# KieDani/UpliftingTableTennis

Hardware: AMD Instinct MI355X
Metric: frames/sec end-to-end (detect+uplift), 1280x720 (higher is better)
Workload: dtype bf16

## Files before the change

### upliftingtabletennis_amd/csrc/conv.h

```cpp
#pragma once
#include "common.h"
#include "wasb_graph.h"

namespace ttup {

struct PackedConv {
    int cout = 0, cin_total = 0, c0 = 0, k = 1, stride = 1, ck = 32;
    void*  w_dev = nullptr;
    void*  w3_dev = nullptr;
    int    mt3 = 0;
    float* bias_dev = nullptr;
    size_t w_bytes = 0;
};

struct Roi {
    int y0 = 0, y1 = 0, x0 = 0, x1 = 0;
    int sy0 = 0, sy1 = 0, sx0 = 0, sx1 = 0;
    const int* flag = nullptr;
    __host__ __device__ bool outside(int f, int y, int x) const {
        if (f == 2 && sy1 > 0) return y < sy0 || y >= sy1 || x < sx0 || x >= sx1;
        return y < y0 || y >= y1 || x < x0 || x >= x1;
    }
};

struct ConvLaunch {
    const void* src0 = nullptr;
    const void* src1 = nullptr;
    const void* residual = nullptr;
    void* dst = nullptr;
    int batch = 0, h = 0, w = 0;
    int relu = 0;
    const PackedConv* follow = nullptr;
    void* dst2 = nullptr;
    const void* res2 = nullptr;
    const void* res3 = nullptr; int sh3 = 0;
    const int* n_active = nullptr;
    Roi roi;
    const PackedConv* lin16 = nullptr; void* lin16_dst = nullptr;
    const PackedConv* lin32 = nullptr; void* lin32_dst = nullptr;
    const PackedConv* pair = nullptr; void* pair_dst = nullptr; int pair_relu = 0;
};

int pack_conv(const FoldedConv& a, const FoldedConv* b , int cin_pad, int dtype, PackedConv* out);
void free_conv(PackedConv* p);

int launch_conv(const PackedConv& p, const ConvLaunch& l, int dtype, hipStream_t stream);
bool conv_f32_mfma_supported(const PackedConv& p);
int launch_conv_f32_mfma(const PackedConv& p, const ConvLaunch& l, hipStream_t stream);
bool conv_x3_supported(const PackedConv& p);
int launch_conv_x3(const PackedConv& p, const ConvLaunch& l, hipStream_t stream);
int pack_conv_x3(const std::vector<float>& w_tap_cin_cout, int cout, int cin_total, int c0, int k, int stride, PackedConv* out);

int launch_stem(const PackedConv& p1, const PackedConv& p2, const PackedConv& p3, const void* x0, void* t2, void* a1,
                int batch, int h, int w, hipStream_t st, int frames_per_sample = 0);
#define TTUP_LAYOUT_NHWC4_FRAME 2

int launch_bneck_trans(const PackedConv& p1, const PackedConv& p5, const PackedConv& p6, const void* a2, const void* t2,
                       void* b0, void* b1, int batch, int h, int w, hipStream_t st);

struct BBSum {
    const void* terms[3] = {nullptr, nullptr, nullptr}; int shifts[3] = {0, 0, 0}; int n_terms = 0;
    void* ysum = nullptr;
    float* heat = nullptr; const float* head_w = nullptr; float head_bias = 0.f; float* pv = nullptr; long long* pi = nullptr;
};
int bb_chain_tiles_per_img(int h, int w);
int launch_bb_chain(const PackedConv* const* convs, int n_convs, const void* x, void* y, int batch, int h, int w,
                    const PackedConv* follow, void* y_follow, hipStream_t st, const BBSum* sum = nullptr);

int launch_upsum(const void* base, const void* const* terms, const int* shifts, int n_terms, void* dst,
                 int batch, int h, int w, int c, int dtype, hipStream_t stream, const int* n_active = nullptr, const Roi* roi = nullptr);

int launch_nchw_to_nhwc(const float* src, void* dst, int batch, int cin, int cpad, int h, int w, int dtype, hipStream_t stream);
int launch_nhwc_to_nchw(const void* src, float* dst, int batch, int c, int h, int w, int dtype, hipStream_t stream);

int launch_head(const void* src, const float* w_dev, const float* bias_dev, int n_out, float* heat, int batch, int h, int w, int cin,
                int dtype, hipStream_t stream, const int* n_active = nullptr, const Roi* roi = nullptr);

int launch_preprocess(const uint8_t* frames, int n_frames, int src_h, int src_w, int dst_h, int dst_w,
                      void* out, int out_layout, int dtype, int first_triple, int n_triples, int frames_per_sample, hipStream_t stream);

int launch_preprocess_crops(const uint8_t* frames, int n_frames, int src_h, int src_w, int dst_h, int dst_w, float* out,
                            const int* crops_dev, int crop0, const int* n_active_dev, int max_crops, int crop_h, int crop_w,
                            int frames_per_sample, hipStream_t stream);

}
```

### upliftingtabletennis_amd/csrc/conv.hip

```cpp
#include "conv_mfma.h"
#include "conv64.h"
#include "conv_stem.h"
#include "conv_bneck.h"
#include "conv_bb.h"
#include "chain16.h"
#include "conv_pointwise.h"

namespace ttup {

int launch_stem(const PackedConv& p1, const PackedConv& p2, const PackedConv& p3, const void* x0, void* t2, void* a1,
                int batch, int h, int w, hipStream_t st, int frames_per_sample) {
    TTUP_REQUIRE((p1.cout == 64 && p1.cin_total == 16 && p1.k == 3 && p1.stride == 1 && p1.ck == 16) ||
                 (p1.cout == 64 && p1.cin_total == 128 && p1.k == 1 && p1.ck == 32), TTUP_EINVAL, "stem: unexpected conv1 shape");
    TTUP_REQUIRE(p2.cout == 64 && p2.cin_total == 64 && p2.k == 3 && p2.stride == 1 && p2.ck == 32, TTUP_EINVAL, "stem: unexpected conv2 shape");
    TTUP_REQUIRE(p3.cout == 32 && p3.cin_total == 64 && p3.k == 1 && p3.ck == 32, TTUP_EINVAL, "stem: unexpected follower shape");
    StemArgs a;
    a.x0 = (const bf16_t*)x0; a.w1 = (const bf16_t*)p1.w_dev; a.b1 = p1.bias_dev; a.w2 = (const bf16_t*)p2.w_dev; a.b2 = p2.bias_dev;
    a.w3 = (const bf16_t*)p3.w_dev; a.b3 = p3.bias_dev; a.t2 = (bf16_t*)t2; a.a1 = (bf16_t*)a1;
    a.H = h; a.W = w; a.tiles_x = cdiv(w, 32); a.tiles_per_img = a.tiles_x * cdiv(h, 8); a.total_tiles = a.tiles_per_img * batch;
    constexpr size_t SMEM = (size_t)(5 * 4 * 64 * 8 + 2 * 9 * 4 * 64 * 8 + 2 * 340 * 32 + 432 * 16) * 2;
    static_assert(SMEM <= 160 * 1024, "LDS budget");
    TTUP_REQUIRE(frames_per_sample == 0 || frames_per_sample == 1 || frames_per_sample == 3, TTUP_EINVAL, "stem: frames per sample must be 0 (X0 records), 1 or 3");
    const bool k4 = p1.k == 1;
    TTUP_REQUIRE(k4 == (frames_per_sample == 3), TTUP_EINVAL, "stem: the 4-step conv1 packing is the three-frame form");
    const dim3 grid(persistent_grid(a.total_tiles));
    if (k4) return launch_noted(stem_kernel<3, true>, grid, 512, SMEM, st, a, "stem_kernel<3, true>");
    if (frames_per_sample == 1) return launch_noted(stem_kernel<1, false>, grid, 512, SMEM, st, a, "stem_kernel<1, false>");
    return launch_noted(stem_kernel<0, false>, grid, 512, SMEM, st, a, "stem_kernel<0, false>");
}

int launch_bneck_trans(const PackedConv& p1, const PackedConv& p5, const PackedConv& p6, const void* a2, const void* t2,
                       void* b0, void* b1, int batch, int h, int w, hipStream_t st) {
    TTUP_REQUIRE(p1.cout == 128 && p1.cin_total == 96 && p1.c0 == 32 && p1.k == 1 && p1.ck == 32, TTUP_EINVAL, "bneck_trans: unexpected conv1 shape");
    TTUP_REQUIRE(p5.cout == 16 && p5.cin_total == 128 && p5.k == 3 && p5.stride == 1 && p5.ck == 32, TTUP_EINVAL, "bneck_trans: unexpected conv5 shape");
    TTUP_REQUIRE(p6.cout == 32 && p6.cin_total == 128 && p6.k == 3 && p6.stride == 2 && p6.ck == 32, TTUP_EINVAL, "bneck_trans: unexpected conv6 shape");
    TTUP_REQUIRE(h % 2 == 0 && w % 2 == 0, TTUP_EINVAL, "bneck_trans: even input size required");
    FusedArgs a;
    a.a2 = (const bf16_t*)a2; a.t2 = (const bf16_t*)t2;
    a.w1 = (const bf16_t*)p1.w_dev; a.b1 = p1.bias_dev; a.w5 = (const bf16_t*)p5.w_dev; a.b5 = p5.bias_dev;
    a.w6 = (const bf16_t*)p6.w_dev; a.b6 = p6.bias_dev; a.b0 = (bf16_t*)b0; a.b1o = (bf16_t*)b1;
    a.H = h; a.W = w; a.tiles_x = cdiv(w, 32); a.tiles_per_img = a.tiles_x * cdiv(h, 8); a.total_tiles = a.tiles_per_img * batch;
    constexpr size_t SMEM = (size_t)(340 * 128 + 3 * 8 * 64 * 8 + 4 * 9 * 64 * 8) * 2 + 512;
    return launch_noted(bneck_trans_kernel, dim3(persistent_grid(a.total_tiles)), 512, SMEM, st, a, "bneck_trans_kernel");
}

constexpr int BB2_TH = 24, BB2_TW = 32;
int bb_chain_tiles_per_img(int h, int w) { return cdiv(w, BB2_TW) * cdiv(h, BB2_TH); }

int launch_bb_chain(const PackedConv* const* convs, int n_convs, const void* x, void* y, int batch, int h, int w,
                    const PackedConv* follow, void* y_follow, hipStream_t st, const BBSum* sum) {
    TTUP_REQUIRE(n_convs == 2 || n_convs == 4, TTUP_EINVAL, "bb_chain: 2 or 4 convs expected");
    const int c = convs[0]->cout;
    BBArgs a;
    a.x = (const bf16_t*)x; a.y = (bf16_t*)y;
    if (sum) {
        TTUP_REQUIRE(c == 16 && n_convs == 4 && sum->n_terms >= 0 && sum->n_terms <= 3, TTUP_EINVAL, "bb_chain: the fused fuse-layer sum rides on the 16-channel two-block chain");
        TTUP_REQUIRE(sum->ysum || (sum->heat && sum->head_w && sum->pv && sum->pi), TTUP_EINVAL, "bb_chain: fused sum needs an output");
        a.nsum = sum->n_terms; a.ysum = (bf16_t*)sum->ysum;
        for (int k = 0; k < sum->n_terms; ++k) { a.st[k] = (const bf16_t*)sum->terms[k]; a.ssh[k] = sum->shifts[k]; }
        a.heat = sum->heat; a.hw = sum->head_w; a.hbias = sum->head_bias; a.pv = sum->pv; a.pi = sum->pi;
    }
    if (follow) {
        TTUP_REQUIRE(c == 32 && n_convs == 2 && follow->cout == 16 && follow->cin_total == 32 && follow->k == 1 && follow->ck == 32 && y_follow, TTUP_EINVAL,
                     "bb_chain: the fused follower is a 1x1 32->16 conv on a 32-channel block");
        a.wf = (const bf16_t*)follow->w_dev; a.bf = follow->bias_dev; a.yf = (bf16_t*)y_follow;
    }
    for (int i = 0; i < n_convs; ++i) {
        const PackedConv& p = *convs[i];
        TTUP_REQUIRE(p.cout == c && p.cin_total == c && p.k == 3 && p.stride == 1 && p.ck == (c == 16 ? 16 : 32), TTUP_EINVAL, "bb_chain: unexpected conv shape");
        a.w[i] = (const bf16_t*)p.w_dev; a.bias[i] = p.bias_dev;
    }
    if (c == 16 && n_convs == 4) {
        static const bool generic = env_set("TTUP_BB2_GENERIC");
        bool shifts_ok = true;
        for (int k = 0; k < a.nsum && k < 3; ++k) shifts_ok = shifts_ok && a.ssh[k] == k + 1;
        const bool sum_stored = !generic && shifts_ok && a.nsum >= 1 && a.nsum <= 3 && a.ysum && !a.heat;
        const bool tail = !generic && shifts_ok && a.nsum == 3 && a.heat && !a.y && !a.ysum;
        const bool plain = !generic && a.nsum == 0 && !a.heat && !a.ysum && a.y;
        if (plain) return launch_c16_t<BB2_TH, BB2_TW, 4>(a, batch, h, w, st);
        if (tail) return launch_c16_t<BB2_TH, BB2_TW, 7>(a, batch, h, w, st);
        if (sum_stored && a.nsum == 1) return launch_c16_t<BB2_TH, BB2_TW, 1>(a, batch, h, w, st);
        if (sum_stored && a.nsum == 2) return launch_c16_t<BB2_TH, BB2_TW, 2>(a, batch, h, w, st);
        if (sum_stored && a.nsum == 3) return launch_c16_t<BB2_TH, BB2_TW, 3>(a, batch, h, w, st);
        return launch_bb2_t<16, BB2_TH, BB2_TW>(a, batch, h, w, st);
    }
    if (c == 16 && n_convs == 2) return launch_bb_t<16, 8, 32>(a, batch, h, w, st);
    if (c == 32 && n_convs == 2) {
        return launch_bb_t<32, 22, 30>(a, batch, h, w, st);
    }
    set_error("bb_chain: C=%d with %d convs unsupported", c, n_convs);
    return TTUP_EINVAL;
}

void free_conv(PackedConv* p) {
    if (p->w_dev) (void)hipFree(p->w_dev);
    if (p->bias_dev) (void)hipFree(p->bias_dev);
    if (p->w3_dev) (void)hipFree(p->w3_dev);
    p->w_dev = nullptr; p->bias_dev = nullptr; p->w3_dev = nullptr;
}

int pack_conv(const FoldedConv& a, const FoldedConv* b, int cin_pad, int dtype, PackedConv* out) {
    const int k = a.k, taps = k * k, cout = a.cout;
    const int c0 = cin_pad > a.cin ? cin_pad : a.cin;
    const int c1 = b ? b->cin : 0;
    TTUP_REQUIRE(!b || (b->cout == cout && b->k == k && k == 1), TTUP_EINVAL, "two-source conv needs matching 1x1 convs");
    TTUP_REQUIRE(cout % 16 == 0 && cout <= 128, TTUP_EINVAL, "cout %d unsupported", cout);
    const int cin_total = c0 + c1;
    out->cout = cout; out->cin_total = cin_total; out->c0 = c0; out->k = k; out->stride = a.stride;
    std::vector<float> bias(cout);
    for (int i = 0; i < cout; ++i) bias[i] = a.bias[i] + (b ? b->bias[i] : 0.f);
    auto wval = [&](int co, int ci, int tap) -> float {
        if (ci < c0) return ci < a.cin ? a.w[((size_t)co * a.cin + ci) * taps + tap] : 0.f;
        return b->w[((size_t)co * b->cin + (ci - c0)) * taps + tap];
    };
    TTUP_HIP_CHECK(hipMalloc((void**)&out->bias_dev, cout * sizeof(float)));
    TTUP_HIP_CHECK(hipMemcpy(out->bias_dev, bias.data(), cout * sizeof(float), hipMemcpyHostToDevice));
    if (dtype == TTUP_DTYPE_F32) {
        std::vector<float> w((size_t)taps * cin_total * cout);
        for (int t = 0; t < taps; ++t)
            for (int ci = 0; ci < cin_total; ++ci)
                for (int co = 0; co < cout; ++co) w[((size_t)t * cin_total + ci) * cout + co] = wval(co, ci, t);
        out->w_bytes = w.size() * sizeof(float);
        out->ck = 0;
        TTUP_HIP_CHECK(hipMalloc(&out->w_dev, out->w_bytes));
        TTUP_HIP_CHECK(hipMemcpy(out->w_dev, w.data(), out->w_bytes, hipMemcpyHostToDevice));
        return pack_conv_x3(w, cout, cin_total, c0, k, a.stride, out);
    }
    TTUP_REQUIRE(c0 % 16 == 0 && c1 % 32 == 0, TTUP_EINVAL, "channel counts %d+%d unsupported", c0, c1);
    int ck = (c0 % 32 == 0) ? 32 : 16;
    TTUP_REQUIRE(ck == 32 || (c1 == 0 && k == 3), TTUP_EINVAL, "16-channel chunks only for single-source 3x3");
    const int mt = cout / 16, ksteps = ck == 32 ? taps : (taps + 1) / 2, nchunk = cin_total / ck;
    std::vector<bf16_t> w((size_t)nchunk * ksteps * mt * 64 * 8);
    size_t idx = 0;
    for (int c = 0; c < nchunk; ++c)
        for (int s = 0; s < ksteps; ++s)
            for (int m = 0; m < mt; ++m)
                for (int l = 0; l < 64; ++l) {
                    const int i = l & 15, g = l >> 4;
                    const int co = (i >> 2) * (4 * mt) + m * 4 + (i & 3);
                    for (int j = 0; j < 8; ++j) {
                        int tap, ci;
                        if (ck == 32) { tap = s; ci = c * 32 + 8 * g + j; }
                        else { tap = 2 * s + (g >> 1); ci = c * 16 + 8 * (g & 1) + j; }
                        w[idx++] = f32_to_bf16(tap < taps ? wval(co, ci, tap) : 0.f);
                    }
                }
    out->ck = ck;
    out->w_bytes = w.size() * sizeof(bf16_t);
    TTUP_HIP_CHECK(hipMalloc(&out->w_dev, out->w_bytes));
    TTUP_HIP_CHECK(hipMemcpy(out->w_dev, w.data(), out->w_bytes, hipMemcpyHostToDevice));
    return TTUP_OK;
}

int launch_conv(const PackedConv& p, const ConvLaunch& l, int dtype, hipStream_t st) {
    if (dtype == TTUP_DTYPE_F32) {
        TTUP_REQUIRE(!l.res2 && !l.res3, TTUP_EINVAL, "conv: extra fuse-layer terms are a bf16-path fusion");
        static const bool direct = env_set("TTUP_F32_DIRECT");
        static const bool exact = env_set("TTUP_F32_EXACT");
        if (!direct && !exact && conv_x3_supported(p)) return launch_conv_x3(p, l, st);
        if (!direct && conv_f32_mfma_supported(p)) return launch_conv_f32_mfma(p, l, st);
        TTUP_REQUIRE(!l.n_active, TTUP_EINVAL, "conv: a device-side batch needs the matrix-pipe fp32 kernel");
        ConvFArgs a;
        a.src0 = (const float*)l.src0; a.src1 = (const float*)l.src1; a.w = (const float*)p.w_dev; a.bias = p.bias_dev;
        a.residual = (const float*)l.residual; a.dst = (float*)l.dst;
        a.c0 = p.c0; a.c1 = p.cin_total - p.c0; a.cout = p.cout; a.ks = p.k; a.stride = p.stride;
        a.H = l.h; a.W = l.w; a.OH = (l.h + p.stride - 1) / p.stride; a.OW = (l.w + p.stride - 1) / p.stride; a.relu = l.relu;
        a.total = (long long)l.batch * a.OH * a.OW * a.cout;
        const int threads = 256;
        const long long blocks = (a.total + threads - 1) / threads;
        kernel_note("conv_direct_f32_kernel");
        hipLaunchKernelGGL(conv_direct_f32_kernel, dim3((unsigned)blocks), dim3(threads), 0, st, a);
        TTUP_LAUNCH_CHECK();
        return TTUP_OK;
    }
    TTUP_REQUIRE(!(l.res2 || l.res3) || (p.stride == 2 && !l.follow), TTUP_EINVAL, "conv: extra fuse-layer terms ride on the stride-2 chain convs only");
    if (l.follow) {
        TTUP_REQUIRE(p.k == 3 && p.stride == 1 && p.ck == 32 && p.cout == 64, TTUP_EINVAL, "conv: fused follower needs a 3x3 s1 conv with 64 outputs");
        return launch_mfma<32, 64, 3, 1, 8, 32, 8, true>(p, l, st);
    }
    if (p.k == 3 && p.stride == 1 && p.ck == 32 && p.cout == 64 && p.cin_total == 64 && p.c0 == 64 && !l.src1) return launch_conv64(p, l, st);
    if (l.pair) return launch_s2_pair(p, l, st);
    TTUP_REQUIRE(!l.lin16 && !l.lin32, TTUP_EINVAL, "conv: linear 1x1 followers ride on the 64 -> 64 3x3 kernel only");
    if (p.k == 3 && p.stride == 1) return p.ck == 32 ? dispatch_cout<32, 3, 1, 8, 32>(p, l, st) : dispatch_cout<16, 3, 1, 8, 32>(p, l, st);
    if (p.k == 3 && p.stride == 2) return p.ck == 32 ? dispatch_cout<32, 3, 2, 4, 32>(p, l, st) : dispatch_cout<16, 3, 2, 4, 32>(p, l, st);
    if (p.k == 1 && p.stride == 1 && p.ck == 32) return dispatch_cout<32, 1, 1, 8, 32>(p, l, st);
    set_error("conv: k=%d stride=%d ck=%d unsupported", p.k, p.stride, p.ck);
    return TTUP_EINVAL;
}

int launch_upsum(const void* base, const void* const* terms, const int* shifts, int n_terms, void* dst,
                 int batch, int h, int w, int c, int dtype, hipStream_t stream, const int* n_active, const Roi* roi) {
    UpsumArgs a;
    a.base = base; a.n = n_terms; a.dst = dst; a.H = h; a.W = w; a.C = c; a.batch = batch;
    if (roi) a.roi = *roi;
    TTUP_REQUIRE(!a.roi.flag || dtype == TTUP_DTYPE_F32, TTUP_EINVAL, "upsum: output regions are an fp32-path feature");
    for (int k = 0; k < 3; ++k) { a.t[k] = k < n_terms ? terms[k] : nullptr; a.shift[k] = k < n_terms ? shifts[k] : 0; }
    a.total = (long long)batch * h * w * c;
    a.n_active = n_active; a.per_sample = (long long)h * w * c;
    if (a.total == 0) return TTUP_OK;
    long long blocks = (a.total + 255) / 256;
    if (n_active && blocks > 8192) blocks = 8192;
    TTUP_REQUIRE(!n_active || dtype == TTUP_DTYPE_F32, TTUP_EINVAL, "upsum: a device-side batch is an fp32-path feature");
    kernel_note(dtype == TTUP_DTYPE_F32 ? "upsum_kernel<float>" : c % 8 == 0 ? "upsum_bf16x8_kernel" : "upsum_kernel<bf16>");
    if (dtype == TTUP_DTYPE_F32) hipLaunchKernelGGL(upsum_kernel<float>, dim3((unsigned)blocks), dim3(256), 0, stream, a);
    else if (c % 8 == 0) {
        a.total /= 8;
        hipLaunchKernelGGL(upsum_bf16x8_kernel, dim3((unsigned)((a.total + 255) / 256)), dim3(256), 0, stream, a);
    } else hipLaunchKernelGGL(upsum_kernel<bf16_t>, dim3((unsigned)blocks), dim3(256), 0, stream, a);
    TTUP_LAUNCH_CHECK();
    return TTUP_OK;
}

int launch_nchw_to_nhwc(const float* src, void* dst, int batch, int cin, int cpad, int h, int w, int dtype, hipStream_t stream) {
    const long long total = (long long)batch * h * w * cpad;
    const unsigned blocks = (unsigned)((total + 255) / 256);
    if (dtype == TTUP_DTYPE_F32) hipLaunchKernelGGL(nchw_to_nhwc_kernel<float>, dim3(blocks), dim3(256), 0, stream, src, (float*)dst, cin, cpad, h * w, total);
    else hipLaunchKernelGGL(nchw_to_nhwc_kernel<bf16_t>, dim3(blocks), dim3(256), 0, stream, src, (bf16_t*)dst, cin, cpad, h * w, total);
    TTUP_LAUNCH_CHECK();
    return TTUP_OK;
}

int launch_nhwc_to_nchw(const void* src, float* dst, int batch, int c, int h, int w, int dtype, hipStream_t stream) {
    const long long total = (long long)batch * h * w * c;
    const unsigned blocks = (unsigned)((total + 255) / 256);
    if (dtype == TTUP_DTYPE_F32) hipLaunchKernelGGL(nhwc_to_nchw_kernel<float>, dim3(blocks), dim3(256), 0, stream, (const float*)src, dst, c, h * w, total);
    else hipLaunchKernelGGL(nhwc_to_nchw_kernel<bf16_t>, dim3(blocks), dim3(256), 0, stream, (const bf16_t*)src, dst, c, h * w, total);
    TTUP_LAUNCH_CHECK();
    return TTUP_OK;
}

int launch_head(const void* src, const float* w_dev, const float* bias_dev, int n_out, float* heat, int batch, int h, int w, int cin, int dtype,
                hipStream_t stream, const int* n_active, const Roi* roi) {
    const Roi r = roi ? *roi : Roi();
    TTUP_REQUIRE(cin == 16, TTUP_EINVAL, "head expects 16 input channels, got %d", cin);
    const long long hw = (long long)h * w, npix = (long long)batch * hw;
    if (npix == 0) return TTUP_OK;
    long long blocks = (npix + 255) / 256;
    if (n_active && blocks > 8192) blocks = 8192;
    if (dtype == TTUP_DTYPE_F32) hipLaunchKernelGGL((head_kernel<float, 16>), dim3((unsigned)blocks), dim3(256), 0, stream, (const float*)src, w_dev, bias_dev, n_out, heat, hw, npix, n_active, r, w);
    else hipLaunchKernelGGL((head_kernel<bf16_t, 16>), dim3((unsigned)blocks), dim3(256), 0, stream, (const bf16_t*)src, w_dev, bias_dev, n_out, heat, hw, npix, n_active, r, w);
    TTUP_LAUNCH_CHECK();
    return TTUP_OK;
}

int launch_preprocess(const uint8_t* frames, int n_frames, int src_h, int src_w, int dst_h, int dst_w,
                      void* out, int out_layout, int dtype, int first_triple, int n_triples, int frames_per_sample, hipStream_t stream) {
    TTUP_REQUIRE(frames_per_sample == 1 || frames_per_sample == 3, TTUP_EINVAL, "frames_per_sample must be 1 or 3");
    TTUP_REQUIRE(first_triple >= 0 && first_triple + n_triples + frames_per_sample - 1 <= n_frames, TTUP_EINVAL, "sample range outside the clip");
    PreArgs a;
    a.frames = frames; a.out = out; a.src_h = src_h; a.src_w = src_w; a.dst_h = dst_h; a.dst_w = dst_w;
    a.first_triple = first_triple; a.n_triples = n_triples; a.layout = out_layout; a.nf = frames_per_sample;
    a.total = (long long)n_triples * dst_h * dst_w;
    a.scale_x = (double)src_w / dst_w; a.scale_y = (double)src_h / dst_h;
    a.crops = nullptr; a.n_active = nullptr; a.crop0 = 0; a.crop_h = 0; a.crop_w = 0;
    if (a.total == 0) return TTUP_OK;
    if (int rc = device_normalise_lut(&a.lut)) return rc;
    TTUP_REQUIRE(dst_h <= 65535 && n_triples <= 65535, TTUP_EINVAL, "preprocess: grid limit (rows, samples <= 65535)");
    const dim3 grid((unsigned)cdiv(dst_w, 256), (unsigned)dst_h, (unsigned)n_triples);
    TTUP_REQUIRE(out_layout != TTUP_LAYOUT_NHWC4_FRAME || (frames_per_sample == 1 && dtype == TTUP_DTYPE_BF16), TTUP_EINVAL, "per-frame records are bf16, one frame per sample");
    static const bool no_fast = env_set("TTUP_NO_PRE4");
    if (out_layout == TTUP_LAYOUT_NHWC4_FRAME && src_w == dst_w && dst_w % 4 == 0 && ((size_t)frames & 3) == 0 && !no_fast)
        hipLaunchKernelGGL(preprocess_frames4_kernel, dim3((unsigned)cdiv(dst_w, 1024), (unsigned)cdiv(dst_h, PRE4_ROWS), (unsigned)n_triples), dim3(256), 0, stream, a);
    else if ((dtype == TTUP_DTYPE_F32 || out_layout == TTUP_LAYOUT_NCHW_F32) && out_layout != TTUP_LAYOUT_NHWC4_FRAME)
        hipLaunchKernelGGL(preprocess_kernel<float>, grid, dim3(256), 0, stream, a);
    else
        hipLaunchKernelGGL(preprocess_kernel<bf16_t>, grid, dim3(256), 0, stream, a);
    TTUP_LAUNCH_CHECK();
    return TTUP_OK;
}

int launch_preprocess_crops(const uint8_t* frames, int n_frames, int src_h, int src_w, int dst_h, int dst_w, float* out,
                            const int* crops_dev, int crop0, const int* n_active_dev, int max_crops, int crop_h, int crop_w,
                            int frames_per_sample, hipStream_t stream) {
    PreArgs a;
    a.frames = frames; a.out = out; a.src_h = src_h; a.src_w = src_w; a.dst_h = dst_h; a.dst_w = dst_w;
    a.first_triple = 0; a.n_triples = n_frames - frames_per_sample + 1; a.layout = TTUP_LAYOUT_NHWC16; a.nf = frames_per_sample;
    a.total = (long long)max_crops * crop_h * crop_w;
    a.scale_x = (double)src_w / dst_w; a.scale_y = (double)src_h / dst_h;
    a.crops = crops_dev; a.n_active = n_active_dev; a.crop0 = crop0; a.crop_h = crop_h; a.crop_w = crop_w;
    if (a.total == 0) return TTUP_OK;
    if (int rc = device_normalise_lut(&a.lut)) return rc;
    TTUP_REQUIRE(a.total < (1ll << 32), TTUP_EINVAL, "preprocess crops: more than 2^32 crop pixels");
    hipLaunchKernelGGL(preprocess_kernel<float>, dim3((unsigned)((a.total + 255) / 256)), dim3(256), 0, stream, a);
    TTUP_LAUNCH_CHECK();
    return TTUP_OK;
}

}
```

### upliftingtabletennis_amd/csrc/conv_bneck.h

```cpp
#pragma once
#include "conv_dev.h"
#include "conv.h"

namespace ttup {

struct FusedArgs {
    const bf16_t* a2 = nullptr; const bf16_t* t2 = nullptr;
    const bf16_t* w1 = nullptr; const float* b1 = nullptr;
    const bf16_t* w5 = nullptr; const float* b5 = nullptr;
    const bf16_t* w6 = nullptr; const float* b6 = nullptr;
    bf16_t* b0 = nullptr; bf16_t* b1o = nullptr;
    int H = 0, W = 0, tiles_x = 0, tiles_per_img = 0, total_tiles = 0;
};

__device__ __forceinline__ int l1_off(int pix, int c8) { return pix * 128 + ((c8 ^ (pix & 15)) << 3); }
__device__ __forceinline__ int st_off(int pix, int c8) { return pix * 32 + ((c8 ^ ((4 - ((pix >> 2) & 3)) & 3)) << 3); }

__global__ __launch_bounds__(512) void bneck_trans_kernel(FusedArgs a) {
    constexpr int IH = 10, IW = 34, NPIX = IH * IW;
    constexpr int NT1 = 22;
    constexpr int W1_U = 3 * 8 * 64, W5_U = 4 * 9 * 64;
    extern __shared__ __attribute__((aligned(16))) char smem[];
    bf16_t* s_l1 = (bf16_t*)smem;
    bf16_t* s_w1 = s_l1 + NPIX * 128;
    bf16_t* s_w5 = s_w1 + W1_U * 8;
    float* s_b1 = (float*)(s_w5 + W5_U * 8);
    const int tid = threadIdx.x, lane = tid & 63, wave = tid >> 6;
    const int n = lane & 15, g = lane >> 4;
    StageRegs<W1_U> w1regs; StageRegs<W5_U> w5regs;
    stage_load_512<W1_U>(w1regs, a.w1, tid);
    stage_load_512<W5_U>(w5regs, a.w5, tid);
    const float b1v = tid < 128 ? a.b1[tid] : 0.f;
    const int cc = wave & 3, m6 = wave >> 2;
    bf16x8 af6[9];
#pragma unroll
    for (int s9 = 0; s9 < 9; ++s9) af6[s9] = *(const bf16x8*)(a.w6 + (((cc * 9 + s9) * 2 + m6) * 64 + lane) * 8);
    const f32x4 bias6 = *(const f32x4*)(a.b6 + g * 8 + m6 * 4);
    const f32x4 b5 = *(const f32x4*)(a.b5 + g * 4);
    const int my_tiles = (a.total_tiles - (int)blockIdx.x + (int)gridDim.x - 1) / (int)gridDim.x;

    u32x4 pb[3][3];
    bool p_in[3];
    unsigned pyx[3];
#pragma unroll
    for (int t = 0; t < 3; ++t) {
        int pix = (wave + 8 * t) * 16 + n;
        pix = pix < NPIX ? pix : NPIX - 1;
        pyx[t] = (unsigned)((pix / IW) << 8 | (pix % IW));
    }
    unsigned poff[3];
#pragma unroll
    for (int t = 0; t < 3; ++t) poff[t] = (unsigned)(((pyx[t] >> 8) * a.W + (pyx[t] & 255u)) * 64 + g * 16);
    auto issue_pix = [&](int it) {
        const TileAt t = tile_at<8, 32, 1>(xcd_tile(blockIdx.x + it * gridDim.x, a.total_tiles), a.tiles_per_img, a.tiles_x);
        const int b = t.b, gy0 = t.y0, gx0 = t.x0;
        if (gy0 >= 0 && gy0 + IH <= a.H && gx0 >= 0 && gx0 + IW <= a.W) {
            const size_t gp0 = (size_t)(b * a.H + gy0) * a.W + gx0;
            const char* base_a = (const char*)(a.a2 + gp0 * 32);
            const char* base_t = (const char*)(a.t2 + gp0 * 64);
#pragma unroll
            for (int t = 0; t < 3; ++t) {
                p_in[t] = wave + 8 * t < NT1;
                const unsigned o = opaque_u32(poff[t]), o2 = o * 2u - (unsigned)(g * 16);
                pb[t][0] = *(const u32x4*)(base_a + o);
                pb[t][1] = *(const u32x4*)(base_t + o2);
                pb[t][2] = *(const u32x4*)(base_t + o2 + 64);
            }
            return;
        }
#pragma unroll
        for (int t = 0; t < 3; ++t) {
            const int j = wave + 8 * t;
            unsigned q = pyx[t];
            asm volatile("" : "+v"(q));
            const int gy = gy0 + (int)(q >> 8), gx = gx0 + (int)(q & 255u);
            p_in[t] = j < NT1 && gy >= 0 && gy < a.H && gx >= 0 && gx < a.W;
            const size_t gp = (size_t)(b * a.H + gy) * a.W + gx;
#pragma unroll
            for (int c = 0; c < 3; ++c) {
                pb[t][c] = u32x4{0u, 0u, 0u, 0u};
                if (p_in[t]) pb[t][c] = (c == 0) ? *(const u32x4*)(a.a2 + gp * 32 + g * 8) : *(const u32x4*)(a.t2 + gp * 64 + (c - 1) * 32 + g * 8);
            }
        }
    };
    if (my_tiles <= 0) return;
    issue_pix(0);
    stage_store_512<W1_U>(s_w1, w1regs, tid);
    stage_store_512<W5_U>(s_w5, w5regs, tid);
    if (tid < 128) s_b1[tid] = b1v;
    prefetch_arrived(pb[0]); prefetch_arrived(pb[1]); prefetch_arrived(pb[2]);

    for (int it = 0; it < my_tiles; ++it) {
        const TileAt tile = tile_at<8, 32>(xcd_tile(blockIdx.x + it * gridDim.x, a.total_tiles), a.tiles_per_img, a.tiles_x);
        const int b = tile.b, oy0 = tile.y0, ox0 = tile.x0;
        __syncthreads();
        bf16x8 afp[2][2];
        f32x4 bqp[2][2];
        auto load_w1 = [&](int st, bf16x8 (&a2)[2]) __attribute__((always_inline)) {
            const int q = st / 3, chunk = st % 3;
            a2[0] = *(const bf16x8*)(s_w1 + ((chunk * 8 + 2 * q) * 64 + lane) * 8);
            a2[1] = *(const bf16x8*)(s_w1 + ((chunk * 8 + 2 * q + 1) * 64 + lane) * 8);
        };
        auto load_bq = [&](int q, f32x4 (&b2)[2]) __attribute__((always_inline)) {
            b2[0] = *(const f32x4*)(s_b1 + g * 32 + q * 8); b2[1] = *(const f32x4*)(s_b1 + g * 32 + q * 8 + 4);
        };
        load_w1(0, afp[0]);
        load_bq(0, bqp[0]);
#pragma unroll
        for (int q = 0; q < 4; ++q) {
            f32x4 acc[3][2];
            const f32x4 bq0 = bqp[q & 1][0], bq1 = bqp[q & 1][1];
#pragma unroll
            for (int t = 0; t < 3; ++t) { acc[t][0] = bq0; acc[t][1] = bq1; }
#pragma unroll
            for (int chunk = 0; chunk < 3; ++chunk) {
                const int st = q * 3 + chunk;
                if (st + 1 < 12) load_w1(st + 1, afp[(st + 1) & 1]);
                if (chunk == 0 && q + 1 < 4) load_bq(q + 1, bqp[(q + 1) & 1]);
                __builtin_amdgcn_sched_barrier(0);
                const bf16x8 af0 = afp[st & 1][0], af1 = afp[st & 1][1];
#pragma unroll
                for (int t = 0; t < 3; ++t) {
                    if (wave + 8 * t >= NT1) continue;
                    const bf16x8 bfr = __builtin_bit_cast(bf16x8, pb[t][chunk]);
                    acc[t][0] = __builtin_amdgcn_mfma_f32_16x16x32_bf16(af0, bfr, acc[t][0], 0, 0, 0);
                    acc[t][1] = __builtin_amdgcn_mfma_f32_16x16x32_bf16(af1, bfr, acc[t][1], 0, 0, 0);
                }
                __builtin_amdgcn_sched_barrier(0);
            }
#pragma unroll
            for (int t = 0; t < 3; ++t) {
                const int j = wave + 8 * t, pix = j * 16 + n;
                if (j >= NT1 || pix >= NPIX) continue;
                const bool inside = p_in[t];
                u32x4 pk;
#pragma unroll
                for (int i = 0; i < 4; ++i) {
                    const unsigned w = relu_pk(pack2(acc[t][i >> 1][2 * (i & 1)], acc[t][i >> 1][2 * (i & 1) + 1]));
                    pk[i] = inside ? w : 0u;
                }
                *(u32x4*)(s_l1 + l1_off(pix, g * 4 + q)) = pk;
            }
        }
        __syncthreads();
        if (it + 1 < my_tiles) issue_pix(it + 1);
        {
            const int q2 = wave >> 1, ch = wave & 1;
            f32x4 acc[2] = {b5, b5};
            bf16x8 brow[2][4], af[2][3];
            unsigned bt[9];
            {
                const int P0 = (2 * q2) * IW + ch * 16 + n;
#pragma unroll
                for (int t = 0; t < 9; ++t) bt[t] = (unsigned)(P0 * 256) + (unsigned)(((g ^ ((P0 + t) & 15)) & 15) << 4);
            }
            auto load_group = [&](int j, bf16x8 (&br)[4], bf16x8 (&a3)[3]) __attribute__((always_inline)) {
                const int c = j / 3, dx = j % 3;
#pragma unroll
                for (int rr = 0; rr < 4; ++rr) br[rr] = *(const bf16x8*)((const char*)s_l1 + (bt[2 * rr + dx] ^ (unsigned)(c << 6)) + (rr * IW + dx) * 256);
#pragma unroll
                for (int dy = 0; dy < 3; ++dy) a3[dy] = *(const bf16x8*)(s_w5 + ((c * 9 + dy * 3 + dx) * 64 + lane) * 8);
            };
            load_group(0, brow[0], af[0]);
#pragma unroll
            for (int j = 0; j < 12; ++j) {
                if (j + 1 < 12) load_group(j + 1, brow[(j + 1) & 1], af[(j + 1) & 1]);
                __builtin_amdgcn_sched_barrier(0);
#pragma unroll
                for (int dy = 0; dy < 3; ++dy) {
                    acc[0] = __builtin_amdgcn_mfma_f32_16x16x32_bf16(af[j & 1][dy], brow[j & 1][dy], acc[0], 0, 0, 0);
                    acc[1] = __builtin_amdgcn_mfma_f32_16x16x32_bf16(af[j & 1][dy], brow[j & 1][dy + 1], acc[1], 0, 0, 0);
                }
                __builtin_amdgcn_sched_barrier(0);
            }
#pragma unroll
            for (int t = 0; t < 2; ++t) {
                const int oy = oy0 + 2 * q2 + t, ox = ox0 + ch * 16 + n;
                if (oy < a.H && ox < a.W)
                    *(u32x2*)(a.b0 + ((size_t)(b * a.H + oy) * a.W + ox) * 16 + g * 4) =
                        u32x2{relu_pk(pack2(acc[t][0], acc[t][1])), relu_pk(pack2(acc[t][2], acc[t][3]))};
            }
        }
        f32x4 part[4];
        {
            const f32x4 seed = cc == 0 ? bias6 : f32x4{0.f, 0.f, 0.f, 0.f};
#pragma unroll
            for (int r = 0; r < 4; ++r) part[r] = seed;
#pragma unroll
            for (int s9 = 0; s9 < 9; ++s9) {
                const int dy = s9 / 3, dx = s9 % 3;
#pragma unroll
                for (int r = 0; r < 4; ++r) {
                    const int pix = (2 * r + dy) * IW + 2 * n + dx;
                    const bf16x8 bfr = *(const bf16x8*)(s_l1 + l1_off(pix, cc * 4 + g));
                    part[r] = __builtin_amdgcn_mfma_f32_16x16x32_bf16(af6[s9], bfr, part[r], 0, 0, 0);
                }
            }
        }
        __syncthreads();
        {
            float* s_part = (float*)s_l1;
#pragma unroll
            for (int r = 0; r < 4; ++r) *(f32x4*)(s_part + (((m6 * 4 + cc) * 4 + r) * 64 + lane) * 4) = part[r];
        }
        __syncthreads();
        {
            const float* s_part = (const float*)s_l1;
            const int mr = wave >> 2, rr = wave & 3;
            f32x4 v = *(const f32x4*)(s_part + (((mr * 4 + 0) * 4 + rr) * 64 + lane) * 4);
#pragma unroll
            for (int c = 1; c < 4; ++c) v += *(const f32x4*)(s_part + (((mr * 4 + c) * 4 + rr) * 64 + lane) * 4);
            const int OH = (a.H + 1) >> 1, OW = (a.W + 1) >> 1;
            const int oy = (oy0 >> 1) + rr, ox = (ox0 >> 1) + n;
            prefetch_arrived(pb[0]); prefetch_arrived(pb[1]); prefetch_arrived(pb[2]);
            if (oy < OH && ox < OW)
                *(u32x2*)(a.b1o + ((size_t)(b * OH + oy) * OW + ox) * 32 + g * 8 + mr * 4) = u32x2{relu_pk(pack2(v[0], v[1])), relu_pk(pack2(v[2], v[3]))};
        }
    }
}

}
```

### upliftingtabletennis_amd/csrc/conv_stem.h

```cpp
#pragma once
#include "conv64.h"

namespace ttup {

struct StemArgs {
    const bf16_t* x0 = nullptr;
    const bf16_t* w1 = nullptr; const float* b1 = nullptr;
    const bf16_t* w2 = nullptr; const float* b2 = nullptr;
    const bf16_t* w3 = nullptr; const float* b3 = nullptr;
    bf16_t* t2 = nullptr; bf16_t* a1 = nullptr;
    int H = 0, W = 0, tiles_x = 0, tiles_per_img = 0, total_tiles = 0;
};

template <int NF, bool K4 = false>
__global__ __launch_bounds__(512) void stem_kernel(StemArgs a) {
    static_assert(!K4 || NF == 3, "the 4-step conv1 is the three-frame form");
    constexpr int XH = 12, XW = 36, TH1 = 10, TW1 = 34, NP1 = TH1 * TW1;
    constexpr int KS1 = K4 ? 4 : 5;
    constexpr int XS = K4 ? 12 : 16;
    constexpr int W1_U = KS1 * 4 * 64, W2_U = 2 * 9 * 4 * 64;
    constexpr int X_UNITS = NF ? XH * XW * NF : XH * XW * 2;
    constexpr int X_PT = (X_UNITS + 511) / 512;
    extern __shared__ __attribute__((aligned(16))) char smem[];
    bf16_t* s_w1 = (bf16_t*)smem;
    bf16_t* s_w2 = s_w1 + W1_U * 8;
    bf16_t* s_t1 = s_w2 + W2_U * 8;
    bf16_t* s_x = s_t1 + 2 * NP1 * 32;
    const int tid = threadIdx.x, lane = tid & 63, wave = tid >> 6;
    const int n = lane & 15, g = lane >> 4;
    StageRegs<W1_U> w1regs; StageRegs<W2_U> w2regs;
    stage_load_512<W1_U>(w1regs, a.w1, tid);
    stage_load_512<W2_U>(w2regs, a.w2, tid);
    bf16x8 af3[2][2];
#pragma unroll
    for (int k = 0; k < 2; ++k)
#pragma unroll
        for (int m = 0; m < 2; ++m) af3[k][m] = follower_frag<2>(a.w3, k, m, n, g);
    f32x4 b1[4], b2[4], b3[2];
#pragma unroll
    for (int m = 0; m < 4; ++m) { b1[m] = *(const f32x4*)(a.b1 + g * 16 + m * 4); b2[m] = *(const f32x4*)(a.b2 + g * 16 + m * 4); }
#pragma unroll
    for (int m = 0; m < 2; ++m) b3[m] = *(const f32x4*)(a.b3 + g * 8 + m * 4);
    int koff1[KS1];
#pragma unroll
    for (int s5 = 0; s5 < KS1; ++s5) {
        if (K4) {
            const int kk0 = 32 * s5 + 8 * g, r = kk0 / 40, o0 = kk0 % 40;
            koff1[s5] = r < 3 ? r * XW * XS + o0 : 0;
        } else {
            int tap = 2 * s5 + (g >> 1); tap = tap > 8 ? 8 : tap; koff1[s5] = ((tap / 3) * XW + tap % 3) * 16 + (g & 1) * 8;
        }
    }
    const bf16_t* bB[3];
#pragma unroll
    for (int dx = 0; dx < 3; ++dx) bB[dx] = s_t1 + lds_off<32, TW1>(0, n + dx, g);

    const int my_tiles = (a.total_tiles - (int)blockIdx.x + (int)gridDim.x - 1) / (int)gridDim.x;
    u32x4 px[NF ? 1 : 2];
    u32x2 pf[NF ? X_PT : 1];
    if (NF) {
        for (int u = tid; u < (K4 ? (XH * XW * XS * 2 + 16) / 16 : XH * XW * 2); u += 512) ((u32x4*)s_x)[u] = u32x4{0u, 0u, 0u, 0u};
        __syncthreads();
    }
    unsigned xoff[NF ? X_PT : 1];
    if constexpr (NF != 0) {
#pragma unroll
        for (int k = 0; k < X_PT; ++k) {
            const int u = tid + k * 512;
            const int f = u % (NF ? NF : 1), pix = u / (NF ? NF : 1);
            xoff[k] = u < X_UNITS ? (unsigned)(((f * a.H + pix / XW) * a.W + pix % XW) * 8) : 0u;
        }
    }
    auto issue = [&](int it) {
        const TileAt t = tile_at<8, 32, 2>(xcd_tile(blockIdx.x + it * gridDim.x, a.total_tiles), a.tiles_per_img, a.tiles_x);
        const int b = t.b, gy0 = t.y0, gx0 = t.x0;
        if (NF) {
            if (gy0 >= 0 && gy0 + XH <= a.H && gx0 >= 0 && gx0 + XW <= a.W) {
                const char* base = (const char*)(a.x0 + (((size_t)b * a.H + gy0) * a.W + gx0) * 4);
#pragma unroll
                for (int k = 0; k < X_PT; ++k) pf[k] = *(const u32x2*)(base + opaque_u32(xoff[k]));
                return;
            }
#pragma unroll
            for (int k = 0; k < X_PT; ++k) {
                const int u = tid + k * 512;
                const int f = u % (NF ? NF : 1), pix = u / (NF ? NF : 1);
                const int gy = gy0 + pix / XW, gx = gx0 + pix % XW;
                pf[k] = u32x2{0u, 0u};
                if (u < X_UNITS && gy >= 0 && gy < a.H && gx >= 0 && gx < a.W)
                    pf[k] = *(const u32x2*)(a.x0 + (((size_t)(b + f) * a.H + gy) * a.W + gx) * 4);
            }
            return;
        }
#pragma unroll
        for (int k = 0; k < 2; ++k) {
            const int u = tid + k * 512;
            const int c8 = u & 1, pix = u >> 1;
            const int gy = gy0 + pix / XW, gx = gx0 + pix % XW;
            px[k & (NF ? 0 : 1)] = u32x4{0u, 0u, 0u, 0u};
            if (u < X_UNITS && gy >= 0 && gy < a.H && gx >= 0 && gx < a.W)
                px[k & (NF ? 0 : 1)] = *(const u32x4*)(a.x0 + ((size_t)(b * a.H + gy) * a.W + gx) * 16 + c8 * 8);
        }
    };
    auto commit = [&]() {
        if (NF) {
#pragma unroll
            for (int k = 0; k < X_PT; ++k) {
                const int u = tid + k * 512;
                if (u < X_UNITS) *(u32x2*)(s_x + (u / (NF ? NF : 1)) * XS + (u % (NF ? NF : 1)) * 4) = pf[k];
            }
        } else {
#pragma unroll
            for (int k = 0; k < 2; ++k) { const int u = tid + k * 512; if (u < X_UNITS) ((u32x4*)s_x)[u] = px[k & (NF ? 0 : 1)]; }
        }
    };
    auto epilogue = [&](const f32x4 (&acc)[4][2], int b, int oy0, int ox0) __attribute__((always_inline)) {
#pragma unroll
        for (int t = 0; t < 2; ++t) {
            const int r = 2 * (wave >> 1) + t, cg = wave & 1;
            const int oy = oy0 + r, ox = ox0 + cg * 16 + n;
            const bool ok = oy < a.H && ox < a.W;
            u32x4 pk[2];
#pragma unroll
            for (int q = 0; q < 2; ++q) {
                pk[q] = pack8(acc[2 * q][t], acc[2 * q + 1][t], true);
                if (ok) *(u32x4*)(a.t2 + ((size_t)(b * a.H + oy) * a.W + ox) * 64 + g * 16 + q * 8) = pk[q];
            }
            f32x4 c3[2] = {b3[0], b3[1]};
#pragma unroll
            for (int k = 0; k < 2; ++k)
#pragma unroll
                for (int m = 0; m < 2; ++m) c3[m] = __builtin_amdgcn_mfma_f32_16x16x32_bf16(af3[k][m], __builtin_bit_cast(bf16x8, pk[k]), c3[m], 0, 0, 0);
            if (ok) *(u32x4*)(a.a1 + ((size_t)(b * a.H + oy) * a.W + ox) * 32 + g * 8) = pack8(c3[0], c3[1], true);
        }
    };
    constexpr bool STAGGER = K4;
    const bool late = __builtin_amdgcn_readfirstlane(wave) >= 4;
    f32x4 acc[4][2];
    int eb = 0, eoy0 = 0, eox0 = 0;
    bool pending = false;
    if (my_tiles <= 0) return;
    issue(0);
    stage_store_512<W1_U>(s_w1, w1regs, tid);
    stage_store_512<W2_U>(s_w2, w2regs, tid);
    commit();
    if (my_tiles > 1) issue(1);
    for (int it = 0; it < my_tiles; ++it) {
        const TileAt tile = tile_at<8, 32>(xcd_tile(blockIdx.x + it * gridDim.x, a.total_tiles), a.tiles_per_img, a.tiles_x);
        const int b = tile.b, oy0 = tile.y0, ox0 = tile.x0;
        const bool t1_inside = oy0 >= 1 && oy0 + 9 <= a.H && ox0 >= 1 && ox0 + 33 <= a.W;
        __syncthreads();
#pragma unroll
        for (int t = 0; t < 3; ++t) {
            const int j = wave + 8 * t;
            if (j >= 22) continue;
            const int p = j * 16 + n, pc = p < NP1 ? p : NP1 - 1;
            const int y = pc / TW1, x = pc % TW1;
            const bf16_t* xb = s_x + (y * XW + x) * XS;
            f32x4 acc[4] = {b1[0], b1[1], b1[2], b1[3]};
#pragma unroll
            for (int s5 = 0; s5 < KS1; ++s5) {
                bf16x8 bfr;
                if (K4) {
                    const u32x2 lo = *(const u32x2*)(xb + koff1[s5]), hi = *(const u32x2*)(xb + koff1[s5] + 4);
                    bfr = __builtin_bit_cast(bf16x8, u32x4{lo.x, lo.y, hi.x, hi.y});
                } else bfr = *(const bf16x8*)(xb + koff1[s5]);
#pragma unroll
                for (int m = 0; m < 4; ++m) {
                    const bf16x8 af = *(const bf16x8*)(s_w1 + ((s5 * 4 + m) * 64 + lane) * 8);
                    acc[m] = __builtin_amdgcn_mfma_f32_16x16x32_bf16(af, bfr, acc[m], 0, 0, 0);
                }
            }
            if (p < NP1) {
                const int gy = oy0 - 1 + y, gx = ox0 - 1 + x;
#pragma unroll
                for (int q = 0; q < 2; ++q) {
                    u32x4 pk = pack8(acc[2 * q], acc[2 * q + 1], true);
                    if (!t1_inside) {
                        const bool inside = gy >= 0 && gy < a.H && gx >= 0 && gx < a.W;
#pragma unroll
                        for (int i = 0; i < 4; ++i) pk[i] = inside ? pk[i] : 0u;
                    }
                    *(u32x4*)(s_t1 + (g >> 1) * (NP1 * 32) + lds_off<32, TW1>(y, x, (g & 1) * 2 + q)) = pk;
                }
            }
        }
        __syncthreads();
        commit();
        if (it + 2 < my_tiles) issue(it + 2);
        if (STAGGER && late && pending) epilogue(acc, eb, eoy0, eox0);
#pragma unroll
        for (int m = 0; m < 4; ++m) { acc[m][0] = b2[m]; acc[m][1] = b2[m]; }
        static_assert(TW1 == 34 && NP1 == 340, "conv64_tile_mfma's tile");
        conv64_tile_mfma(acc, bB, s_w2, wave, lane);
        if (STAGGER && late) { eb = b; eoy0 = oy0; eox0 = ox0; pending = true; }
        else epilogue(acc, b, oy0, ox0);
    }
    if (STAGGER && late && pending) epilogue(acc, eb, eoy0, eox0);
}

}
```

### upliftingtabletennis_amd/csrc/wasb_net.h

```cpp
#pragma once
#include "conv.h"

namespace ttup {
size_t upsum_head_ws_bytes(int n_maps, int H, int W);
int launch_upsum_head(const void* base, const void* const* terms, const int* shifts, int n_terms, const float* w_dev, float bias,
                      float* heat, int n_maps, int H, int W, long long* argmax, float* win, void* ws, size_t ws_bytes, hipStream_t st);
int refine_argmax(const float* heat, int n_maps, int H, int W, long long* argmax, float* win, void* ws, size_t ws_bytes, hipStream_t st);
int launch_argmax_finish(const float* heat, int n_maps, int H, int W, int nblk, const float* pv, const long long* pi, long long* argmax, float* win, hipStream_t st);

struct Tensor : TensorShape { void* ptr = nullptr; };

struct CertState {
    bool enabled = false;
    float eps = 0.f;
    static constexpr float GUARD = 1.25f;
    int R = 72;
    int small = 0;
    int K = 256;
    int maxc = 8;
    int maxf = 8;
    int CH = 0, nchunks = 0, max_crops = 0, Hc = 0, Wc = 0;
    int budget = 0;
    bool exact_windows = false;
    int audit_mod = 0, audit_phase = 0;
    struct ::ttup_wasb* cropnet = nullptr;
    struct Slot {
        int* cand_idx = nullptr; int* cand_cnt = nullptr; int* cand_crop = nullptr; float* cand_val = nullptr; float* cand_win = nullptr;
        float* cand_bf = nullptr;
        int* guard_cnt = nullptr;
        int* crop_rec = nullptr; int* n_crops = nullptr; int* n_active = nullptr; int* status = nullptr;
        int* roi_flag = nullptr;
        float* margin = nullptr;
        hipEvent_t done = nullptr;
        hipEvent_t read_status = nullptr, read_info = nullptr, read_margin = nullptr;
    } slot[2];
    int cur = 0;
    unsigned long long* stats = nullptr;
    float* crop_heat = nullptr;
    hipStream_t stream = nullptr;
    hipEvent_t lanes_done = nullptr;
};
}

struct ttup_wasb {
    int H = 0, W = 0, max_batch = 0, dtype = 0, micro = 1, in_ch = 9;
    std::vector<ttup::PackedConv> convs;
    std::vector<ttup::Tensor> tensors;
    std::vector<ttup::Op> ops;
    std::map<std::string, int> taps;
    int t_input = -1, t_out = -1;
    int t_frames = -1;
    bool frames_mode = false;
    float* head_w_dev = nullptr; float* head_b_dev = nullptr; float head_bias = 0.f;
    int n_out = 1;
    float* heat_scratch = nullptr;
    void* refine_ws = nullptr; size_t refine_ws_bytes = 0;
    long long* argmax_scratch = nullptr; float* win_scratch = nullptr;
    int last_batch = 0;
    bool fused_head = false;
    const int* n_active = nullptr;
    std::vector<ttup::Roi> op_roi; ttup::Roi out_roi; const int* roi_flag = nullptr;
    std::vector<char> blob;
    ttup::CertState cert;
    struct Lane {
        std::vector<void*> ptr;
        float* heat_scratch = nullptr; void* refine_ws = nullptr; long long* argmax_scratch = nullptr; float* win_scratch = nullptr;
        hipStream_t stream = nullptr; hipEvent_t done = nullptr;
    };
    std::vector<Lane> lanes;
    hipEvent_t fork = nullptr;
    hipEvent_t pass_done = nullptr;
    bool pass_recorded = false;

    void use_lane(int l) {
        const Lane& L = lanes[l];
        for (size_t i = 0; i < tensors.size(); ++i) tensors[i].ptr = L.ptr[i];
        heat_scratch = L.heat_scratch; refine_ws = L.refine_ws; argmax_scratch = L.argmax_scratch; win_scratch = L.win_scratch;
    }
    size_t esize() const { return dtype == TTUP_DTYPE_F32 ? 4 : 2; }
    ~ttup_wasb();
};

namespace ttup {
int run_ops(ttup_wasb* net, int mb, hipStream_t st);
int compute_roi(ttup_wasb* net, int lo, int hi, int lo2 = 0, int hi2 = 0);
void cert_free(ttup_wasb* net);
int cert_begin(ttup_wasb* net, int batch, hipStream_t caller);
int cert_scan(ttup_wasb* net, const float* heat, const long long* argmax, int b0, int mb, hipStream_t st);
int cert_finish(ttup_wasb* net, const float* x_dev, const uint8_t* frames_dev, int n_frames, int src_h, int src_w, int batch,
                int64_t* argmax_dev, float* win_dev, hipStream_t caller);
}
```

### upliftingtabletennis_amd/csrc/wasb_net.hip

```cpp
#include "wasb_net.h"
#include "wasb_blob.h"
#include <string.h>
#include <stdlib.h>
#include <memory>

using namespace ttup;

ttup_wasb::~ttup_wasb() {
    cert_free(this);
    for (auto& c : convs) free_conv(&c);
    for (auto& L : lanes) {
        for (void* q : L.ptr) if (q) (void)hipFree(q);
        if (L.heat_scratch) (void)hipFree(L.heat_scratch);
        if (L.refine_ws) (void)hipFree(L.refine_ws);
        if (L.argmax_scratch) (void)hipFree(L.argmax_scratch);
        if (L.win_scratch) (void)hipFree(L.win_scratch);
        if (L.stream) (void)hipStreamDestroy(L.stream);
        if (L.done) (void)hipEventDestroy(L.done);
    }
    if (fork) (void)hipEventDestroy(fork);
    if (pass_done) (void)hipEventDestroy(pass_done);
    if (head_w_dev) (void)hipFree(head_w_dev);
    if (head_b_dev) (void)hipFree(head_b_dev);
}

namespace {

void chain_args(const ttup_wasb* net, const Op& op, const PackedConv* cv[4], BBSum* sum) {
    for (int k = 0; k < 4; ++k) cv[k] = k < op.n_chain ? &net->convs[op.chain[k]] : nullptr;
    sum->n_terms = op.n_terms;
    for (int k = 0; k < op.n_terms; ++k) { sum->terms[k] = net->tensors[op.terms[k]].ptr; sum->shifts[k] = op.shifts[k]; }
}

int run_op(ttup_wasb* net, const Op& op, int mb, hipStream_t st) {
    if (op.kind == Op::CONV) {
        const Tensor& s = net->tensors[op.src0];
        ConvLaunch l;
        l.src0 = s.ptr; l.src1 = op.src1 >= 0 ? net->tensors[op.src1].ptr : nullptr;
        l.residual = op.residual >= 0 ? net->tensors[op.residual].ptr : nullptr;
        l.dst = net->tensors[op.dst].ptr; l.batch = mb; l.h = s.h; l.w = s.w; l.relu = op.relu; l.n_active = net->n_active;
        if (!net->op_roi.empty() && net->roi_flag) { l.roi = net->op_roi[&op - net->ops.data()]; l.roi.flag = net->roi_flag; }
        if (op.conv2 >= 0) { l.follow = &net->convs[op.conv2]; l.dst2 = net->tensors[op.dst2].ptr; }
        if (op.lin16 >= 0) { l.lin16 = &net->convs[op.lin16]; l.lin16_dst = net->tensors[op.lin16_dst].ptr; }
        if (op.lin32 >= 0) { l.lin32 = &net->convs[op.lin32]; l.lin32_dst = net->tensors[op.lin32_dst].ptr; }
        if (op.pair >= 0) { l.pair = &net->convs[op.pair]; l.pair_dst = net->tensors[op.pair_dst].ptr; l.pair_relu = op.pair_relu; }
        if (op.res2 >= 0) l.res2 = net->tensors[op.res2].ptr;
        if (op.res3 >= 0) { l.res3 = net->tensors[op.res3].ptr; l.sh3 = op.sh3; }
        const int rc = launch_conv(net->convs[op.conv], l, net->dtype, st);
        if (rc) return rc;
    } else if (op.kind == Op::STEM) {
        const Tensor& s = net->tensors[op.src0];
        const bool fm = net->frames_mode && net->t_frames >= 0 && op.conv1f >= 0;
        const int rc = launch_stem(net->convs[fm ? op.conv1f : op.conv], net->convs[op.conv2], net->convs[op.conv3], fm ? net->tensors[net->t_frames].ptr : s.ptr,
                                   net->tensors[op.dst].ptr, net->tensors[op.dst2].ptr, mb, s.h, s.w, st, fm ? net->in_ch / 3 : 0);
        if (rc) return rc;
    } else if (op.kind == Op::UPSUM_HEAD) {
        return TTUP_OK;
    } else if (op.kind == Op::BB_CHAIN) {
        if (op.head) return TTUP_OK;
        const Tensor& s = net->tensors[op.src0];
        const PackedConv* cv[4]; BBSum sum;
        chain_args(net, op, cv, &sum);
        int rc;
        if (op.n_chain == 4 && op.n_terms > 0) {
            sum.ysum = net->tensors[op.dst2].ptr;
            rc = launch_bb_chain(cv, 4, s.ptr, op.dst >= 0 ? net->tensors[op.dst].ptr : nullptr, mb, s.h, s.w, nullptr, nullptr, st, &sum);
        } else {
            rc = launch_bb_chain(cv, op.n_chain, s.ptr, net->tensors[op.dst].ptr, mb, s.h, s.w,
                                 op.conv2 >= 0 ? &net->convs[op.conv2] : nullptr, op.dst2 >= 0 ? net->tensors[op.dst2].ptr : nullptr, st);
        }
        if (rc) return rc;
    } else if (op.kind == Op::BNECK_TRANS) {
        const Tensor& s = net->tensors[op.src0];
        const int rc = launch_bneck_trans(net->convs[op.conv], net->convs[op.conv2], net->convs[op.conv3], s.ptr, net->tensors[op.src1].ptr,
                                          net->tensors[op.dst].ptr, net->tensors[op.dst2].ptr, mb, s.h, s.w, st);
        if (rc) return rc;
    } else {
        const Tensor& d = net->tensors[op.dst];
        const void* terms[3] = {nullptr, nullptr, nullptr};
        for (int k = 0; k < op.n_terms; ++k) terms[k] = net->tensors[op.terms[k]].ptr;
        Roi roi;
        if (!net->op_roi.empty() && net->roi_flag) { roi = net->op_roi[&op - net->ops.data()]; roi.flag = net->roi_flag; }
        const int rc = launch_upsum(net->tensors[op.src0].ptr, terms, op.shifts, op.n_terms, d.ptr, mb, d.h, d.w, d.c, net->dtype, st, net->n_active, &roi);
        if (rc) return rc;
    }
    return TTUP_OK;
}

int run_graph(ttup_wasb* net, int mb, hipStream_t st) {
    for (const Op& op : net->ops) { const int rc = run_op(net, op, mb, st); if (rc) return rc; }
    return TTUP_OK;
}

int run_head_op(ttup_wasb* net, int mb, float* heat, long long* am, float* wn, hipStream_t st) {
    const Op& op = net->ops.back();
    if (op.kind == Op::BB_CHAIN) {
        const Tensor& s = net->tensors[op.src0];
        const int nblk = bb_chain_tiles_per_img(s.h, s.w);
        TTUP_REQUIRE(net->refine_ws && net->refine_ws_bytes >= (size_t)mb * nblk * 12, TTUP_EINVAL, "head: workspace too small");
        const PackedConv* cv[4]; BBSum sum;
        chain_args(net, op, cv, &sum);
        sum.heat = heat; sum.head_w = net->head_w_dev; sum.head_bias = net->head_bias;
        sum.pi = (long long*)net->refine_ws; sum.pv = (float*)(sum.pi + (size_t)mb * nblk);
        int rc = launch_bb_chain(cv, 4, s.ptr, nullptr, mb, s.h, s.w, nullptr, nullptr, st, &sum);
        if (rc) return rc;
        if (am || wn) {
            TTUP_REQUIRE(am && wn, TTUP_EINVAL, "head: argmax and window outputs come together");
            rc = launch_argmax_finish(heat, mb, s.h, s.w, nblk, sum.pv, sum.pi, am, wn, st);
        }
        return rc;
    }
    const void* terms[3] = {nullptr, nullptr, nullptr};
    for (int k = 0; k < op.n_terms; ++k) terms[k] = net->tensors[op.terms[k]].ptr;
    return launch_upsum_head(net->tensors[op.src0].ptr, terms, op.shifts, op.n_terms, net->head_w_dev, net->head_bias, heat, mb, net->H, net->W,
                             am, wn, net->refine_ws, net->refine_ws_bytes, st);
}

int forward_micro(ttup_wasb* net, const float* x_dev, const uint8_t* frames_dev, int n_frames, int src_h, int src_w, int batch, int b0,
                  float* heat_dev, int64_t* argmax_dev, float* win_dev, int lane, hipStream_t st) {
    const int H = net->H, W = net->W;
    const size_t hw = (size_t)H * W;
    const int K = net->n_out;
    const int mb = batch - b0 < net->micro ? batch - b0 : net->micro;
    net->use_lane(lane);
    int rc;
    const int nf = net->in_ch / 3;
    net->frames_mode = !x_dev && net->t_frames >= 0;
    if (x_dev) rc = launch_nchw_to_nhwc(x_dev + (size_t)b0 * net->in_ch * hw, net->tensors[net->t_input].ptr, mb, net->in_ch, 16, H, W, net->dtype, st);
    else if (net->frames_mode)
        rc = launch_preprocess(frames_dev, n_frames, src_h, src_w, H, W, net->tensors[net->t_frames].ptr, TTUP_LAYOUT_NHWC4_FRAME, net->dtype, b0, mb + nf - 1, 1, st);
    else rc = launch_preprocess(frames_dev, n_frames, src_h, src_w, H, W, net->tensors[net->t_input].ptr, TTUP_LAYOUT_NHWC16, net->dtype, b0, mb, nf, st);
    if (rc) return rc;
    rc = run_graph(net, mb, st);
    if (rc) return rc;
    float* heat = heat_dev ? heat_dev + (size_t)b0 * K * hw : net->heat_scratch;
    if (net->fused_head) {
        const bool peaks = argmax_dev || win_dev;
        long long* am = peaks ? (argmax_dev ? (long long*)argmax_dev + b0 : net->argmax_scratch) : nullptr;
        float* wn = peaks ? (win_dev ? win_dev + (size_t)b0 * 9 : net->win_scratch) : nullptr;
        rc = run_head_op(net, mb, heat, am, wn, st);
        if (rc) return rc;
        if (net->cert.enabled && argmax_dev && win_dev) return cert_scan(net, heat, am, b0, mb, st);
        return TTUP_OK;
    }
    rc = launch_head(net->tensors[net->t_out].ptr, net->head_w_dev, net->head_b_dev, K, heat, mb, H, W, 16, net->dtype, st, net->n_active);
    if (rc) return rc;
    if (argmax_dev || win_dev) {
        long long* am = argmax_dev ? (long long*)argmax_dev + (size_t)b0 * K : net->argmax_scratch;
        float* wn = win_dev ? win_dev + (size_t)b0 * K * 9 : net->win_scratch;
        rc = refine_argmax(heat, mb * K, H, W, am, wn, net->refine_ws, net->refine_ws_bytes, st);
        if (rc) return rc;
        if (net->cert.enabled && argmax_dev && win_dev) return cert_scan(net, heat, am, b0, mb, st);
    }
    return TTUP_OK;
}

int forward_impl(ttup_wasb* net, const float* x_dev, const uint8_t* frames_dev, int n_frames, int src_h, int src_w,
                 int batch, float* heat_dev, int64_t* argmax_dev, float* win_dev, hipStream_t st) {
    const int n_micro = (batch + net->micro - 1) / net->micro;
    const int n_lanes = n_micro < (int)net->lanes.size() ? (n_micro > 0 ? n_micro : 1) : (int)net->lanes.size();
    const hipStream_t caller = st;
    const bool certify = net->cert.enabled && argmax_dev && win_dev && batch > 0;
    const bool lane_streams = net->lanes[0].stream != nullptr;
    if (!lane_streams && net->pass_recorded) TTUP_HIP_CHECK(hipStreamWaitEvent(caller, net->pass_done, 0));
    if (certify) { const int rc = cert_begin(net, batch, caller); if (rc) return rc; }
    if (lane_streams) {
        TTUP_HIP_CHECK(hipEventRecord(net->fork, caller));
        for (int l = 0; l < n_lanes; ++l) TTUP_HIP_CHECK(hipStreamWaitEvent(net->lanes[l].stream, net->fork, 0));
    }
    int rc_all = TTUP_OK, last_lane = 0;
    for (int b0 = 0, i = 0; b0 < batch && rc_all == TTUP_OK; b0 += net->micro, ++i) {
        rc_all = forward_micro(net, x_dev, frames_dev, n_frames, src_h, src_w, batch, b0, heat_dev, argmax_dev, win_dev,
                               i % n_lanes, lane_streams ? net->lanes[i % n_lanes].stream : caller);
        last_lane = i % n_lanes;
    }
    if (lane_streams) {
        for (int l = 0; l < n_lanes; ++l) {
            (void)hipEventRecord(net->lanes[l].done, net->lanes[l].stream);
            (void)hipStreamWaitEvent(caller, net->lanes[l].done, 0);
        }
    } else if (hipEventRecord(net->pass_done, caller) == hipSuccess) net->pass_recorded = true;
    net->use_lane(last_lane);
    if (rc_all) return rc_all;
    net->last_batch = batch < net->micro ? batch : net->micro;
    if (certify) return cert_finish(net, x_dev, frames_dev, n_frames, src_h, src_w, batch, argmax_dev, win_dev, caller);
    return TTUP_OK;
}

}

namespace ttup {
int run_ops(ttup_wasb* net, int mb, hipStream_t st) { return run_graph(net, mb, st); }

int compute_roi(ttup_wasb* net, int lo, int hi, int lo2, int hi2) {
    TTUP_REQUIRE(net && net->dtype == TTUP_DTYPE_F32 && net->t_out >= 0, TTUP_EINVAL, "compute_roi: an fp32 handle is expected");
    const size_t nt = net->tensors.size();
    struct R { int y0, y1, x0, x1; bool any; };
    auto walk = [&](int l, int h, std::vector<R>& out) -> int {
        std::vector<R> need(nt, R{0, 0, 0, 0, false});
        auto add = [&](int t, int y0, int y1, int x0, int x1) {
            const Tensor& tn = net->tensors[t];
            y0 = y0 < 0 ? 0 : y0; x0 = x0 < 0 ? 0 : x0; y1 = y1 > tn.h ? tn.h : y1; x1 = x1 > tn.w ? tn.w : x1;
            if (y1 <= y0 || x1 <= x0) return;
            R& r = need[t];
            if (!r.any) r = R{y0, y1, x0, x1, true};
            else { r.y0 = y0 < r.y0 ? y0 : r.y0; r.y1 = y1 > r.y1 ? y1 : r.y1; r.x0 = x0 < r.x0 ? x0 : r.x0; r.x1 = x1 > r.x1 ? x1 : r.x1; }
        };
        add(net->t_out, l, h, l, h);
        out.assign(net->ops.size(), R{0, 1, 0, 1, false});
        for (int k = (int)net->ops.size() - 1; k >= 0; --k) {
            const Op& op = net->ops[k];
            TTUP_REQUIRE(op.kind == Op::CONV || op.kind == Op::UPSUM, TTUP_EINVAL, "compute_roi: fused op in an fp32 graph");
            TTUP_REQUIRE(op.conv2 < 0 && op.lin16 < 0 && op.lin32 < 0 && op.pair < 0 && op.res2 < 0 && op.res3 < 0, TTUP_EINVAL, "compute_roi: fused epilogue in an fp32 graph");
            const R d = need[op.dst];
            if (!d.any) continue;
            out[k] = d;
            if (op.kind == Op::CONV) {
                const PackedConv& p = net->convs[op.conv];
                const int s_ = p.stride, pad = p.k / 2;
                add(op.src0, d.y0 * s_ - pad, (d.y1 - 1) * s_ + pad + 1, d.x0 * s_ - pad, (d.x1 - 1) * s_ + pad + 1);
                if (op.src1 >= 0) add(op.src1, d.y0 * s_ - pad, (d.y1 - 1) * s_ + pad + 1, d.x0 * s_ - pad, (d.x1 - 1) * s_ + pad + 1);
                if (op.residual >= 0) add(op.residual, d.y0, d.y1, d.x0, d.x1);
            } else {
                add(op.src0, d.y0, d.y1, d.x0, d.x1);
                for (int j = 0; j < op.n_terms; ++j) { const int sh = op.shifts[j]; add(op.terms[j], d.y0 >> sh, ((d.y1 - 1) >> sh) + 1, d.x0 >> sh, ((d.x1 - 1) >> sh) + 1); }
            }
        }
        return TTUP_OK;
    };
    std::vector<R> r1, r2;
    if (int rc = walk(lo, hi, r1)) return rc;
    const bool two = hi2 > lo2;
    if (two) { if (int rc = walk(lo2, hi2, r2)) return rc; }
    net->op_roi.assign(net->ops.size(), Roi());
    for (size_t k = 0; k < net->ops.size(); ++k) {
        Roi& o = net->op_roi[k];
        o.y0 = r1[k].y0; o.y1 = r1[k].y1; o.x0 = r1[k].x0; o.x1 = r1[k].x1;
        if (two) { o.sy0 = r2[k].y0; o.sy1 = r2[k].y1; o.sx0 = r2[k].x0; o.sx1 = r2[k].x1; }
    }
    if (env_set("TTUP_DEBUG_ROI")) {
        double full = 0, kept = 0, kept2 = 0;
        for (size_t k = 0; k < net->ops.size(); ++k) {
            const Op& op = net->ops[k];
            const Tensor& d = net->tensors[op.dst];
            const Roi& o = net->op_roi[k];
            double w = (double)d.h * d.w;
            if (op.kind == Op::CONV) { const PackedConv& p = net->convs[op.conv]; w *= (double)p.cout * p.cin_total * p.k * p.k; } else w *= d.c;
            full += w; kept += w * ((double)(o.y1 - o.y0) * (o.x1 - o.x0)) / ((double)d.h * d.w);
            kept2 += w * ((double)(o.sy1 - o.sy0) * (o.sx1 - o.sx0)) / ((double)d.h * d.w);
            fprintf(stderr, "roi op %2zu %s dst %3dx%3dx%3d -> [%d,%d)x[%d,%d)  class 2 [%d,%d)x[%d,%d)\n", k, op.kind == Op::CONV ? "conv " : "upsum", d.h, d.w, d.c, o.y0, o.y1, o.x0, o.x1,
                    o.sy0, o.sy1, o.sx0, o.sx1);
        }
        fprintf(stderr, "roi: %.1f %% of the graph's multiply-adds kept (class 2: %.1f %%)\n", 100.0 * kept / full, 100.0 * kept2 / full);
    }
    net->out_roi = Roi();
    net->out_roi.y0 = lo; net->out_roi.y1 = hi; net->out_roi.x0 = lo; net->out_roi.x1 = hi;
    if (two) { net->out_roi.sy0 = lo2; net->out_roi.sy1 = hi2; net->out_roi.sx0 = lo2; net->out_roi.sx1 = hi2; }
    return TTUP_OK;
}
}

int ttup_wasb_create_internal(const void* blob, size_t blob_bytes, int height, int width, int max_batch, int dtype, int micro_override, int lanes_override, ttup_wasb** out) {
    TTUP_REQUIRE(blob && out, TTUP_EINVAL, "ttup_wasb_create: null pointer");
    TTUP_REQUIRE(height > 0 && width > 0 && height % 8 == 0 && width % 8 == 0, TTUP_EINVAL,
                 "ttup_wasb_create: input size %dx%d must be positive multiples of 8", height, width);
    TTUP_REQUIRE(max_batch > 0, TTUP_EINVAL, "ttup_wasb_create: max_batch must be positive");
    TTUP_REQUIRE(dtype == TTUP_DTYPE_BF16 || dtype == TTUP_DTYPE_F32, TTUP_EINVAL, "ttup_wasb_create: unknown dtype %d", dtype);
    std::vector<FoldedConv> folded;
    std::vector<float> head_w, head_b;
    int in_ch = 0, head_out = 0;
    int rc = parse_blob(blob, blob_bytes, &folded, &in_ch, &head_out, &head_w, &head_b);
    if (rc) return rc;
    TTUP_REQUIRE((in_ch == 9 || in_ch == 3) && head_out >= 1 && head_out <= 16, TTUP_EFORMAT, "wasb blob: in_ch=%d head_out=%d unsupported (ball detector 9/3, table detector 3/13)", in_ch, head_out);
    int ndev = 0;
    TTUP_HIP_CHECK(hipGetDeviceCount(&ndev));
    TTUP_REQUIRE(ndev > 0, TTUP_EHIP, "ttup_wasb_create: no HIP device");
    std::unique_ptr<ttup_wasb> net(new ttup_wasb);
    net->H = height; net->W = width; net->max_batch = max_batch; net->dtype = dtype; net->in_ch = in_ch;
    net->blob.assign((const char*)blob, (const char*)blob + blob_bytes);
    net->n_out = head_out == 3 ? 1 : head_out;
    int micro = micro_override > 0 ? micro_override : (int)env_ll("TTUP_MICRO_BATCH", 8);
    if (micro < 1) micro = 1;
    net->micro = micro < max_batch ? micro : max_batch;
    GraphSwitches sw;
    sw.fuse = !env_set("TTUP_NO_FUSE"); sw.fuse_sum = !env_set("TTUP_NO_FUSE_SUM"); sw.fuse_lin = !env_set("TTUP_NO_FUSE_LIN");
    sw.pair = !env_set("TTUP_NO_PAIR"); sw.stem = !env_set("TTUP_NO_STEM"); sw.frames_mode = !env_set("TTUP_NO_FRAMES_MODE");
    const GraphPlan plan = build_graph(folded, in_ch, net->n_out, height, width, net->micro, dtype, sw);
    if (plan.rc) return plan.rc;
    net->ops = plan.ops; net->taps = plan.taps;
    net->t_input = plan.t_input; net->t_out = plan.t_out; net->t_frames = plan.t_frames; net->fused_head = plan.fused_head;
    for (const TensorShape& s : plan.tensors) { Tensor t; static_cast<TensorShape&>(t) = s; net->tensors.push_back(t); }
    for (const ConvRequest& r : plan.convs) {
        net->convs.emplace_back();
        PackedConv& p = net->convs.back();
        rc = pack_conv(plan.source_a(r, folded), r.b >= 0 ? &folded[r.b] : nullptr, r.cin_pad, dtype, &p);
        if (rc) return rc;
        TTUP_REQUIRE(p.cout == r.cout && p.cin_total == r.cin_total && p.c0 == r.c0 && p.k == r.k && p.stride == r.stride, TTUP_EINVAL,
                     "wasb: conv %zu was packed as %d x %d+%d, k %d / s%d; the plan has %d x %d+%d, k %d / s%d", net->convs.size() - 1,
                     p.cout, p.c0, p.cin_total - p.c0, p.k, p.stride, r.cout, r.c0, r.cin_total - r.c0, r.k, r.stride);
    }
    {
        const int first = head_out == 3 ? 1 : 0;
        TTUP_HIP_CHECK(hipMalloc((void**)&net->head_w_dev, (size_t)net->n_out * 16 * sizeof(float)));
        TTUP_HIP_CHECK(hipMemcpy(net->head_w_dev, head_w.data() + (size_t)first * 16, (size_t)net->n_out * 16 * sizeof(float), hipMemcpyHostToDevice));
        TTUP_HIP_CHECK(hipMalloc((void**)&net->head_b_dev, (size_t)net->n_out * sizeof(float)));
        TTUP_HIP_CHECK(hipMemcpy(net->head_b_dev, head_b.data() + first, (size_t)net->n_out * sizeof(float), hipMemcpyHostToDevice));
        net->head_bias = head_b[first];
    }
    const size_t hw = (size_t)height * width;
    net->refine_ws_bytes = ttup_refine_workspace_bytes(net->micro * net->n_out, height, width);
    if (upsum_head_ws_bytes(net->micro, height, width) > net->refine_ws_bytes) net->refine_ws_bytes = upsum_head_ws_bytes(net->micro, height, width);
    {
        int n_lanes = lanes_override > 0 ? lanes_override : (int)env_ll("TTUP_LANES", 2);
        const int n_micro = (max_batch + net->micro - 1) / net->micro;
        if (n_lanes > n_micro) n_lanes = n_micro;
        if (n_lanes < 1) n_lanes = 1;
        if (n_lanes > 4) n_lanes = 4;
        net->lanes.resize(n_lanes);
        for (int l = 0; l < n_lanes; ++l) {
            ttup_wasb::Lane& L = net->lanes[l];
            L.ptr.assign(net->tensors.size(), nullptr);
            for (size_t i = 0; i < net->tensors.size(); ++i) {
                const size_t bytes = plan.tensor_bytes(i);
                if (hipMalloc(&L.ptr[i], bytes) != hipSuccess) { L.ptr[i] = nullptr; set_error("hipMalloc of %zu bytes failed", bytes); return TTUP_ENOMEM; }
            }
            TTUP_HIP_CHECK(hipMalloc((void**)&L.heat_scratch, (size_t)net->micro * net->n_out * hw * sizeof(float)));
            TTUP_HIP_CHECK(hipMalloc(&L.refine_ws, net->refine_ws_bytes));
            TTUP_HIP_CHECK(hipMalloc((void**)&L.argmax_scratch, (size_t)net->micro * net->n_out * sizeof(long long)));
            TTUP_HIP_CHECK(hipMalloc((void**)&L.win_scratch, (size_t)net->micro * net->n_out * 9 * sizeof(float)));
            if (n_lanes > 1) {
                TTUP_HIP_CHECK(hipStreamCreateWithFlags(&L.stream, hipStreamNonBlocking));
                TTUP_HIP_CHECK(hipEventCreateWithFlags(&L.done, hipEventDisableTiming));
            }
        }
        if (n_lanes > 1) TTUP_HIP_CHECK(hipEventCreateWithFlags(&net->fork, hipEventDisableTiming));
        TTUP_HIP_CHECK(hipEventCreateWithFlags(&net->pass_done, hipEventDisableTiming));
        net->use_lane(0);
    }
    if (dtype == TTUP_DTYPE_F32 && env_set("TTUP_DEBUG_FORCE_ROI") && net->H == net->W && net->H >= 2 * 72 + 24) {
        int* flags = nullptr;
        TTUP_HIP_CHECK(hipMalloc((void**)&flags, (size_t)max_batch * sizeof(int)));
        std::vector<int> ones((size_t)max_batch, env_ll("TTUP_DEBUG_FORCE_ROI", 0) == 2 ? 2 : 1);
        TTUP_HIP_CHECK(hipMemcpy(flags, ones.data(), ones.size() * sizeof(int), hipMemcpyHostToDevice));
        if (int rc = compute_roi(net.get(), 72, net->H - 72, 72, 88)) return rc;
        net->roi_flag = flags;
    }
    TTUP_HIP_CHECK(hipDeviceSynchronize());
    *out = net.release();
    return TTUP_OK;
}

extern "C" int ttup_wasb_create(const void* blob, size_t blob_bytes, int height, int width, int max_batch, int dtype, ttup_wasb** out) {
    return ttup_wasb_create_internal(blob, blob_bytes, height, width, max_batch, dtype, 0, 0, out);
}

extern "C" int ttup_wasb_create_ex(const void* blob, size_t blob_bytes, int height, int width, int max_batch, int dtype, int micro_batch, int lanes,
                                   ttup_wasb** out) {
    TTUP_REQUIRE(micro_batch >= 0 && lanes >= 0 && lanes <= 4, TTUP_EINVAL, "ttup_wasb_create_ex: micro_batch %d / lanes %d out of range", micro_batch, lanes);
    return ttup_wasb_create_internal(blob, blob_bytes, height, width, max_batch, dtype, micro_batch, lanes, out);
}

extern "C" int ttup_wasb_streams(ttup_wasb* net, void** out, int cap, int* n_out) {
    TTUP_REQUIRE(net && out && n_out && cap >= 0, TTUP_EINVAL, "ttup_wasb_streams: bad argument");
    int n = 0;
    for (auto& L : net->lanes) if (L.stream && n < cap) out[n++] = (void*)L.stream;
    if (net->cert.enabled && net->cert.stream && n < cap) out[n++] = (void*)net->cert.stream;
    *n_out = n;
    return TTUP_OK;
}

extern "C" void ttup_wasb_destroy(ttup_wasb* net) {
    if (!net) return;
    (void)hipDeviceSynchronize();
    delete net;
}

extern "C" int ttup_wasb_forward(ttup_wasb* net, const float* x_dev, int batch, float* heat_dev, int64_t* argmax_dev, float* win_dev, void* stream) {
    TTUP_REQUIRE(net && x_dev, TTUP_EINVAL, "ttup_wasb_forward: null pointer");
    TTUP_REQUIRE(batch >= 0 && batch <= net->max_batch, TTUP_EINVAL, "ttup_wasb_forward: batch %d outside [0,%d]", batch, net->max_batch);
    return forward_impl(net, x_dev, nullptr, 0, 0, 0, batch, heat_dev, argmax_dev, win_dev, (hipStream_t)stream);
}

extern "C" int ttup_wasb_forward_frames(ttup_wasb* net, const uint8_t* frames_dev, int n_frames, int src_h, int src_w,
                                        float* heat_dev, int64_t* argmax_dev, float* win_dev, void* stream) {
    TTUP_REQUIRE(net && frames_dev, TTUP_EINVAL, "ttup_wasb_forward_frames: null pointer");
    const int nf = net->in_ch / 3;
    TTUP_REQUIRE(n_frames >= nf && src_h > 0 && src_w > 0, TTUP_EINVAL, "ttup_wasb_forward_frames: need at least %d frames", nf);
    const int batch = n_frames - (nf - 1);
    TTUP_REQUIRE(batch <= net->max_batch, TTUP_EINVAL, "ttup_wasb_forward_frames: %d triples exceed max_batch %d", batch, net->max_batch);
    return forward_impl(net, nullptr, frames_dev, n_frames, src_h, src_w, batch, heat_dev, argmax_dev, win_dev, (hipStream_t)stream);
}

extern "C" int ttup_wasb_read_tap(ttup_wasb* net, const char* name, int batch, float* out_dev, int* c, int* h, int* w, void* stream) {
    TTUP_REQUIRE(net && name, TTUP_EINVAL, "ttup_wasb_read_tap: null pointer");
    auto it = net->taps.find(name);
    TTUP_REQUIRE(it != net->taps.end(), TTUP_EINVAL, "ttup_wasb_read_tap: unknown tap '%s'", name);
    const Tensor& t = net->tensors[it->second];
    if (c) *c = t.c; if (h) *h = t.h; if (w) *w = t.w;
    if (!out_dev) return TTUP_OK;
    TTUP_REQUIRE(batch > 0 && batch <= net->micro, TTUP_EINVAL, "ttup_wasb_read_tap: batch %d exceeds the micro-batch %d held in memory", batch, net->micro);
    return launch_nhwc_to_nchw(t.ptr, out_dev, batch, t.c, t.h, t.w, net->dtype, (hipStream_t)stream);
}

#include "wasb_timing.h"

extern "C" int ttup_preprocess_triples(const uint8_t* frames_dev, int n_frames, int src_h, int src_w, int dst_h, int dst_w,
                                       float* out_dev, void* stream) {
    TTUP_REQUIRE(frames_dev && out_dev, TTUP_EINVAL, "ttup_preprocess_triples: null pointer");
    TTUP_REQUIRE(n_frames >= 3 && src_h > 0 && src_w > 0 && dst_h > 0 && dst_w > 0, TTUP_EINVAL, "ttup_preprocess_triples: bad shape");
    return launch_preprocess(frames_dev, n_frames, src_h, src_w, dst_h, dst_w, out_dev, TTUP_LAYOUT_NCHW_F32, TTUP_DTYPE_F32, 0, n_frames - 2, 3, (hipStream_t)stream);
}

extern "C" int ttup_preprocess_frames(const uint8_t* frames_dev, int n_frames, int src_h, int src_w, int dst_h, int dst_w,
                                      float* out_dev, void* stream) {
    TTUP_REQUIRE(frames_dev && out_dev, TTUP_EINVAL, "ttup_preprocess_frames: null pointer");
    TTUP_REQUIRE(n_frames >= 1 && src_h > 0 && src_w > 0 && dst_h > 0 && dst_w > 0, TTUP_EINVAL, "ttup_preprocess_frames: bad shape");
    return launch_preprocess(frames_dev, n_frames, src_h, src_w, dst_h, dst_w, out_dev, TTUP_LAYOUT_NCHW_F32, TTUP_DTYPE_F32, 0, n_frames, 1, (hipStream_t)stream);
}

extern "C" int ttup_wasb_set_priority(ttup_wasb* net, int high) {
    TTUP_REQUIRE(net, TTUP_EINVAL, "ttup_wasb_set_priority: null handle");
    if (net->lanes.size() < 2) return TTUP_OK;
    TTUP_HIP_CHECK(hipDeviceSynchronize());
    int least = 0, greatest = 0;
    TTUP_HIP_CHECK(hipDeviceGetStreamPriorityRange(&least, &greatest));
    for (auto& L : net->lanes) {
        if (L.stream) (void)hipStreamDestroy(L.stream);
        L.stream = nullptr;
        TTUP_HIP_CHECK(hipStreamCreateWithPriority(&L.stream, hipStreamNonBlocking, high ? greatest : least));
    }
    return TTUP_OK;
}

extern "C" int ttup_wasb_micro_batch(ttup_wasb* net) { return net ? net->micro : 0; }
extern "C" int ttup_wasb_out_channels(ttup_wasb* net) { return net ? net->n_out : 0; }
```

Before: 2192.

## Walk persistent tiles in vertical strips and carry halo rows between tiles

The stem and bottleneck-transition kernels now give each persistent workgroup a contiguous run of tiles ordered down image columns, with an XCD-aware slot deal. When the next tile sits directly below the current one, the overlapping halo rows of the first-stage conv output are kept in LDS instead of being recomputed and reloaded. Each carried tile therefore skips part of the first conv's MFMA work and the global loads for those rows. The cost is extra LDS, more complex indexing and some load imbalance from contiguous runs. Env switches can turn off carry and XCD dealing or cap the workgroup count.

```diff
diff --git a/upliftingtabletennis_amd/csrc/conv.h b/upliftingtabletennis_amd/csrc/conv.h
--- a/upliftingtabletennis_amd/csrc/conv.h
+++ b/upliftingtabletennis_amd/csrc/conv.h
@@ -51,12 +51,18 @@
 int launch_conv_x3(const PackedConv& p, const ConvLaunch& l, hipStream_t stream);
 int pack_conv_x3(const std::vector<float>& w_tap_cin_cout, int cout, int cin_total, int c0, int k, int stride, PackedConv* out);
 
+struct StripOpts {
+    bool carry = true;
+    bool xcd_deal = true;
+    int max_wgs = 0;
+};
+
 int launch_stem(const PackedConv& p1, const PackedConv& p2, const PackedConv& p3, const void* x0, void* t2, void* a1,
-                int batch, int h, int w, hipStream_t st, int frames_per_sample = 0);
+                int batch, int h, int w, hipStream_t st, int frames_per_sample = 0, const StripOpts& strip = StripOpts());
 #define TTUP_LAYOUT_NHWC4_FRAME 2
 
 int launch_bneck_trans(const PackedConv& p1, const PackedConv& p5, const PackedConv& p6, const void* a2, const void* t2,
-                       void* b0, void* b1, int batch, int h, int w, hipStream_t st);
+                       void* b0, void* b1, int batch, int h, int w, hipStream_t st, const StripOpts& strip = StripOpts());
 
 struct BBSum {
     const void* terms[3] = {nullptr, nullptr, nullptr}; int shifts[3] = {0, 0, 0}; int n_terms = 0;
diff --git a/upliftingtabletennis_amd/csrc/conv.hip b/upliftingtabletennis_amd/csrc/conv.hip
--- a/upliftingtabletennis_amd/csrc/conv.hip
+++ b/upliftingtabletennis_amd/csrc/conv.hip
@@ -8,8 +8,17 @@
 
 namespace ttup {
 
+static StripWalk strip_walk_for(int batch, int h, int w, const StripOpts& o, int* grid) {
+    StripWalk sw;
+    sw.tiles_x = cdiv(w, 32); sw.tiles_y = cdiv(h, 8); sw.total = sw.tiles_x * sw.tiles_y * batch;
+    sw.xcd_deal = o.xcd_deal; sw.carry = o.carry;
+    *grid = persistent_grid(sw.total);
+    if (o.max_wgs > 0 && *grid > o.max_wgs) *grid = o.max_wgs;
+    return sw;
+}
+
 int launch_stem(const PackedConv& p1, const PackedConv& p2, const PackedConv& p3, const void* x0, void* t2, void* a1,
-                int batch, int h, int w, hipStream_t st, int frames_per_sample) {
+                int batch, int h, int w, hipStream_t st, int frames_per_sample, const StripOpts& strip) {
     TTUP_REQUIRE((p1.cout == 64 && p1.cin_total == 16 && p1.k == 3 && p1.stride == 1 && p1.ck == 16) ||
                  (p1.cout == 64 && p1.cin_total == 128 && p1.k == 1 && p1.ck == 32), TTUP_EINVAL, "stem: unexpected conv1 shape");
     TTUP_REQUIRE(p2.cout == 64 && p2.cin_total == 64 && p2.k == 3 && p2.stride == 1 && p2.ck == 32, TTUP_EINVAL, "stem: unexpected conv2 shape");
@@ -17,20 +26,21 @@
     StemArgs a;
     a.x0 = (const bf16_t*)x0; a.w1 = (const bf16_t*)p1.w_dev; a.b1 = p1.bias_dev; a.w2 = (const bf16_t*)p2.w_dev; a.b2 = p2.bias_dev;
     a.w3 = (const bf16_t*)p3.w_dev; a.b3 = p3.bias_dev; a.t2 = (bf16_t*)t2; a.a1 = (bf16_t*)a1;
-    a.H = h; a.W = w; a.tiles_x = cdiv(w, 32); a.tiles_per_img = a.tiles_x * cdiv(h, 8); a.total_tiles = a.tiles_per_img * batch;
+    int wgs = 0;
+    a.H = h; a.W = w; a.walk = strip_walk_for(batch, h, w, strip, &wgs);
     constexpr size_t SMEM = (size_t)(5 * 4 * 64 * 8 + 2 * 9 * 4 * 64 * 8 + 2 * 340 * 32 + 432 * 16) * 2;
     static_assert(SMEM <= 160 * 1024, "LDS budget");
     TTUP_REQUIRE(frames_per_sample == 0 || frames_per_sample == 1 || frames_per_sample == 3, TTUP_EINVAL, "stem: frames per sample must be 0 (X0 records), 1 or 3");
     const bool k4 = p1.k == 1;
     TTUP_REQUIRE(k4 == (frames_per_sample == 3), TTUP_EINVAL, "stem: the 4-step conv1 packing is the three-frame form");
-    const dim3 grid(persistent_grid(a.total_tiles));
+    const dim3 grid(wgs);
     if (k4) return launch_noted(stem_kernel<3, true>, grid, 512, SMEM, st, a, "stem_kernel<3, true>");
     if (frames_per_sample == 1) return launch_noted(stem_kernel<1, false>, grid, 512, SMEM, st, a, "stem_kernel<1, false>");
     return launch_noted(stem_kernel<0, false>, grid, 512, SMEM, st, a, "stem_kernel<0, false>");
 }
 
 int launch_bneck_trans(const PackedConv& p1, const PackedConv& p5, const PackedConv& p6, const void* a2, const void* t2,
-                       void* b0, void* b1, int batch, int h, int w, hipStream_t st) {
+                       void* b0, void* b1, int batch, int h, int w, hipStream_t st, const StripOpts& strip) {
     TTUP_REQUIRE(p1.cout == 128 && p1.cin_total == 96 && p1.c0 == 32 && p1.k == 1 && p1.ck == 32, TTUP_EINVAL, "bneck_trans: unexpected conv1 shape");
     TTUP_REQUIRE(p5.cout == 16 && p5.cin_total == 128 && p5.k == 3 && p5.stride == 1 && p5.ck == 32, TTUP_EINVAL, "bneck_trans: unexpected conv5 shape");
     TTUP_REQUIRE(p6.cout == 32 && p6.cin_total == 128 && p6.k == 3 && p6.stride == 2 && p6.ck == 32, TTUP_EINVAL, "bneck_trans: unexpected conv6 shape");
@@ -39,9 +49,10 @@
     a.a2 = (const bf16_t*)a2; a.t2 = (const bf16_t*)t2;
     a.w1 = (const bf16_t*)p1.w_dev; a.b1 = p1.bias_dev; a.w5 = (const bf16_t*)p5.w_dev; a.b5 = p5.bias_dev;
     a.w6 = (const bf16_t*)p6.w_dev; a.b6 = p6.bias_dev; a.b0 = (bf16_t*)b0; a.b1o = (bf16_t*)b1;
-    a.H = h; a.W = w; a.tiles_x = cdiv(w, 32); a.tiles_per_img = a.tiles_x * cdiv(h, 8); a.total_tiles = a.tiles_per_img * batch;
-    constexpr size_t SMEM = (size_t)(340 * 128 + 3 * 8 * 64 * 8 + 4 * 9 * 64 * 8) * 2 + 512;
-    return launch_noted(bneck_trans_kernel, dim3(persistent_grid(a.total_tiles)), 512, SMEM, st, a, "bneck_trans_kernel");
+    int wgs = 0;
+    a.H = h; a.W = w; a.walk = strip_walk_for(batch, h, w, strip, &wgs);
+    constexpr size_t SMEM = (size_t)(340 * 128 + 3 * 8 * 64 * 8 + 4 * 9 * 64 * 8) * 2 + 512 + 192;
+    return launch_noted(bneck_trans_kernel, dim3(wgs), 512, SMEM, st, a, "bneck_trans_kernel");
 }
 
 constexpr int BB2_TH = 24, BB2_TW = 32;
diff --git a/upliftingtabletennis_amd/csrc/conv_bneck.h b/upliftingtabletennis_amd/csrc/conv_bneck.h
--- a/upliftingtabletennis_amd/csrc/conv_bneck.h
+++ b/upliftingtabletennis_amd/csrc/conv_bneck.h
@@ -1,6 +1,7 @@
 #pragma once
 #include "conv_dev.h"
 #include "conv.h"
+#include "strip_walk.h"
 
 namespace ttup {
 
@@ -10,7 +11,8 @@
     const bf16_t* w5 = nullptr; const float* b5 = nullptr;
     const bf16_t* w6 = nullptr; const float* b6 = nullptr;
     bf16_t* b0 = nullptr; bf16_t* b1o = nullptr;
-    int H = 0, W = 0, tiles_x = 0, tiles_per_img = 0, total_tiles = 0;
+    int H = 0, W = 0;
+    StripWalk walk;
 };
 
 __device__ __forceinline__ int l1_off(int pix, int c8) { return pix * 128 + ((c8 ^ (pix & 15)) << 3); }
@@ -19,12 +21,19 @@
 __global__ __launch_bounds__(512) void bneck_trans_kernel(FusedArgs a) {
     constexpr int IH = 10, IW = 34, NPIX = IH * IW;
     constexpr int NT1 = 22;
+    constexpr int CARRY_PIX = 2 * IW, CARRY_U = CARRY_PIX * 16;
+    static_assert(CARRY_U == 1024 + 256 / 4, "the carry copy: two 16-byte units per thread and a dword from each of 256 threads");
+    constexpr int CARRY_FROM = (IH - 2) * IW * 16;
+    constexpr int PART_PIX = CARRY_PIX;
+    static_assert(((IH - 2) * IW) % 16 == 0 && (PART_PIX + 128) <= (IH - 2) * IW, "carried rows: same swizzle, clear of the partial sums");
     constexpr int W1_U = 3 * 8 * 64, W5_U = 4 * 9 * 64;
     extern __shared__ __attribute__((aligned(16))) char smem[];
     bf16_t* s_l1 = (bf16_t*)smem;
     bf16_t* s_w1 = s_l1 + NPIX * 128;
     bf16_t* s_w5 = s_w1 + W1_U * 8;
     float* s_b1 = (float*)(s_w5 + W5_U * 8);
+    float* s_b5 = s_b1 + 128;
+    float* s_b6 = s_b5 + 16;
     const int tid = threadIdx.x, lane = tid & 63, wave = tid >> 6;
     const int n = lane & 15, g = lane >> 4;
     StageRegs<W1_U> w1regs; StageRegs<W5_U> w5regs;
@@ -35,33 +44,39 @@
     bf16x8 af6[9];
 #pragma unroll
     for (int s9 = 0; s9 < 9; ++s9) af6[s9] = *(const bf16x8*)(a.w6 + (((cc * 9 + s9) * 2 + m6) * 64 + lane) * 8);
-    const f32x4 bias6 = *(const f32x4*)(a.b6 + g * 8 + m6 * 4);
-    const f32x4 b5 = *(const f32x4*)(a.b5 + g * 4);
-    const int my_tiles = (a.total_tiles - (int)blockIdx.x + (int)gridDim.x - 1) / (int)gridDim.x;
+    const float b56v = tid < 16 ? a.b5[tid] : tid < 48 ? a.b6[tid - 16] : 0.f;
+    const int run_slot = strip_slot((int)blockIdx.x, (int)gridDim.x, a.walk.xcd_deal);
+    const int run_begin = strip_run_begin(run_slot, (int)gridDim.x, a.walk.total);
+    const int my_tiles = strip_run_begin(run_slot + 1, (int)gridDim.x, a.walk.total) - run_begin;
 
     u32x4 pb[3][3];
     bool p_in[3];
-    unsigned pyx[3];
+    auto halo_yx = [&](int t) __attribute__((always_inline)) {
+        const unsigned ti = opaque_u32((unsigned)tid);
+        unsigned pix = ((ti >> 6) + 8u * t) * 16u + (ti & 15u);
+        pix = pix < (unsigned)NPIX ? pix : (unsigned)(NPIX - 1);
+        return (pix / IW) << 8 | (pix % IW);
+    };
+    unsigned poff[3];
 #pragma unroll
     for (int t = 0; t < 3; ++t) {
         int pix = (wave + 8 * t) * 16 + n;
         pix = pix < NPIX ? pix : NPIX - 1;
-        pyx[t] = (unsigned)((pix / IW) << 8 | (pix % IW));
+        poff[t] = (unsigned)(((pix / IW) * a.W + pix % IW) * 64 + g * 16);
     }
-    unsigned poff[3];
-#pragma unroll
-    for (int t = 0; t < 3; ++t) poff[t] = (unsigned)(((pyx[t] >> 8) * a.W + (pyx[t] & 255u)) * 64 + g * 16);
-    auto issue_pix = [&](int it) {
-        const TileAt t = tile_at<8, 32, 1>(xcd_tile(blockIdx.x + it * gridDim.x, a.total_tiles), a.tiles_per_img, a.tiles_x);
-        const int b = t.b, gy0 = t.y0, gx0 = t.x0;
-        if (gy0 >= 0 && gy0 + IH <= a.H && gx0 >= 0 && gx0 + IW <= a.W) {
+    auto issue_pix = [&](const StripTile& st) {
+        const bool carry = st.carry != 0;
+        const int b = st.b, r0 = carry ? 2 : 0, gy0 = st.ty * 8 - 1 + r0, gx0 = st.tx * 32 - 1;
+        if (gy0 >= 0 && gy0 + IH - r0 <= a.H && gx0 >= 0 && gx0 + IW <= a.W) {
             const size_t gp0 = (size_t)(b * a.H + gy0) * a.W + gx0;
             const char* base_a = (const char*)(a.a2 + gp0 * 32);
             const char* base_t = (const char*)(a.t2 + gp0 * 64);
 #pragma unroll
             for (int t = 0; t < 3; ++t) {
-                p_in[t] = wave + 8 * t < NT1;
-                const unsigned o = opaque_u32(poff[t]), o2 = o * 2u - (unsigned)(g * 16);
+                p_in[t] = carry ? (t < 2 || wave < 4) : wave + 8 * t < NT1;
+                if (t == 2 && carry && wave >= 4) continue;
+                const unsigned ln = opaque_u32((unsigned)lane);
+                const unsigned o = t == 2 && carry ? (unsigned)((7 * a.W + 18) * 64) + ((ln & 15u) << 6) + ((ln >> 4) << 4) : opaque_u32(poff[t]), o2 = o * 2u - (unsigned)(g * 16);
                 pb[t][0] = *(const u32x4*)(base_a + o);
                 pb[t][1] = *(const u32x4*)(base_t + o2);
                 pb[t][2] = *(const u32x4*)(base_t + o2 + 64);
@@ -70,11 +85,9 @@
         }
 #pragma unroll
         for (int t = 0; t < 3; ++t) {
-            const int j = wave + 8 * t;
-            unsigned q = pyx[t];
-            asm volatile("" : "+v"(q));
+            const unsigned q = t == 2 && carry ? (7u << 8 | 18u) + (opaque_u32((unsigned)lane) & 15u) : halo_yx(t);
             const int gy = gy0 + (int)(q >> 8), gx = gx0 + (int)(q & 255u);
-            p_in[t] = j < NT1 && gy >= 0 && gy < a.H && gx >= 0 && gx < a.W;
+            p_in[t] = (carry ? (t < 2 || wave < 4) : wave + 8 * t < NT1) && gy >= 0 && gy < a.H && gx >= 0 && gx < a.W;
             const size_t gp = (size_t)(b * a.H + gy) * a.W + gx;
 #pragma unroll
             for (int c = 0; c < 3; ++c) {
@@ -84,15 +97,16 @@
         }
     };
     if (my_tiles <= 0) return;
-    issue_pix(0);
+    StripTile cur = strip_tile_at(a.walk, run_begin, 0);
+    issue_pix(cur);
     stage_store_512<W1_U>(s_w1, w1regs, tid);
     stage_store_512<W5_U>(s_w5, w5regs, tid);
     if (tid < 128) s_b1[tid] = b1v;
+    if (tid < 48) s_b5[tid] = b56v;
     prefetch_arrived(pb[0]); prefetch_arrived(pb[1]); prefetch_arrived(pb[2]);
 
     for (int it = 0; it < my_tiles; ++it) {
-        const TileAt tile = tile_at<8, 32>(xcd_tile(blockIdx.x + it * gridDim.x, a.total_tiles), a.tiles_per_img, a.tiles_x);
-        const int b = tile.b, oy0 = tile.y0, ox0 = tile.x0;
+        const int b = cur.b, oy0 = cur.ty * 8, ox0 = cur.tx * 32;
         __syncthreads();
         bf16x8 afp[2][2];
         f32x4 bqp[2][2];
@@ -104,48 +118,58 @@
         auto load_bq = [&](int q, f32x4 (&b2)[2]) __attribute__((always_inline)) {
             b2[0] = *(const f32x4*)(s_b1 + g * 32 + q * 8); b2[1] = *(const f32x4*)(s_b1 + g * 32 + q * 8 + 4);
         };
-        load_w1(0, afp[0]);
-        load_bq(0, bqp[0]);
-#pragma unroll
-        for (int q = 0; q < 4; ++q) {
-            f32x4 acc[3][2];
-            const f32x4 bq0 = bqp[q & 1][0], bq1 = bqp[q & 1][1];
-#pragma unroll
-            for (int t = 0; t < 3; ++t) { acc[t][0] = bq0; acc[t][1] = bq1; }
-#pragma unroll
-            for (int chunk = 0; chunk < 3; ++chunk) {
-                const int st = q * 3 + chunk;
-                if (st + 1 < 12) load_w1(st + 1, afp[(st + 1) & 1]);
-                if (chunk == 0 && q + 1 < 4) load_bq(q + 1, bqp[(q + 1) & 1]);
-                __builtin_amdgcn_sched_barrier(0);
-                const bf16x8 af0 = afp[st & 1][0], af1 = afp[st & 1][1];
+        {
+            const bool carry = cur.carry != 0;
+            const int pix0 = carry ? CARRY_PIX : 0;
+            const unsigned swz = (unsigned)((g * 4) ^ ((n + (carry ? 4 : 0)) & 15));
+            const int j2 = carry ? 16 : wave + 16;
+            load_w1(0, afp[0]);
+            load_bq(0, bqp[0]);
+#pragma unroll
+            for (int q = 0; q < 4; ++q) {
+                f32x4 acc[3][2];
+                const f32x4 bq0 = bqp[q & 1][0], bq1 = bqp[q & 1][1];
+#pragma unroll
+                for (int t = 0; t < 3; ++t) { acc[t][0] = bq0; acc[t][1] = bq1; }
+                const bool third = carry ? wave == q : wave + 16 < NT1;
+#pragma unroll
+                for (int chunk = 0; chunk < 3; ++chunk) {
+                    const int st = q * 3 + chunk;
+                    if (st + 1 < 12) load_w1(st + 1, afp[(st + 1) & 1]);
+                    if (chunk == 0 && q + 1 < 4) load_bq(q + 1, bqp[(q + 1) & 1]);
+                    __builtin_amdgcn_sched_barrier(0);
+                    const bf16x8 af0 = afp[st & 1][0], af1 = afp[st & 1][1];
+#pragma unroll
+                    for (int t = 0; t < 3; ++t) {
+                        if (t == 2 && !third) continue;
+                        const bf16x8 bfr = __builtin_bit_cast(bf16x8, pb[t][chunk]);
+                        acc[t][0] = __builtin_amdgcn_mfma_f32_16x16x32_bf16(af0, bfr, acc[t][0], 0, 0, 0);
+                        acc[t][1] = __builtin_amdgcn_mfma_f32_16x16x32_bf16(af1, bfr, acc[t][1], 0, 0, 0);
+                    }
+                    __builtin_amdgcn_sched_barrier(0);
+                }
 #pragma unroll
                 for (int t = 0; t < 3; ++t) {
-                    if (wave + 8 * t >= NT1) continue;
-                    const bf16x8 bfr = __builtin_bit_cast(bf16x8, pb[t][chunk]);
-                    acc[t][0] = __builtin_amdgcn_mfma_f32_16x16x32_bf16(af0, bfr, acc[t][0], 0, 0, 0);
-                    acc[t][1] = __builtin_amdgcn_mfma_f32_16x16x32_bf16(af1, bfr, acc[t][1], 0, 0, 0);
-                }
-                __builtin_amdgcn_sched_barrier(0);
-            }
-#pragma unroll
-            for (int t = 0; t < 3; ++t) {
-                const int j = wave + 8 * t, pix = j * 16 + n;
-                if (j >= NT1 || pix >= NPIX) continue;
-                const bool inside = p_in[t];
-                u32x4 pk;
-#pragma unroll
-                for (int i = 0; i < 4; ++i) {
-                    const unsigned w = relu_pk(pack2(acc[t][i >> 1][2 * (i & 1)], acc[t][i >> 1][2 * (i & 1) + 1]));
-                    pk[i] = inside ? w : 0u;
-                }
-                *(u32x4*)(s_l1 + l1_off(pix, g * 4 + q)) = pk;
-            }
-        }
-        __syncthreads();
-        if (it + 1 < my_tiles) issue_pix(it + 1);
+                    const int pix = pix0 + (t < 2 ? wave + 8 * t : j2) * 16 + n;
+                    if (t == 2 && (!third || pix >= NPIX)) continue;
+                    const bool inside = p_in[t];
+                    u32x4 pk;
+#pragma unroll
+                    for (int i = 0; i < 4; ++i) {
+                        const unsigned w = relu_pk(pack2(acc[t][i >> 1][2 * (i & 1)], acc[t][i >> 1][2 * (i & 1) + 1]));
+                        pk[i] = inside ? w : 0u;
+                    }
+                    *(u32x4*)((char*)s_l1 + pix * 256 + ((swz ^ (unsigned)q) << 4)) = pk;
+                }
+            }
+        }
+        __syncthreads();
+        const bool more = it + 1 < my_tiles;
+        const StripTile nxt = more ? strip_tile_at(a.walk, run_begin, it + 1) : cur;
+        if (more) issue_pix(nxt);
         {
             const int q2 = wave >> 1, ch = wave & 1;
+            const f32x4 b5 = *(const f32x4*)(s_b5 + g * 4);
             f32x4 acc[2] = {b5, b5};
             bf16x8 brow[2][4], af[2][3];
             unsigned bt[9];
@@ -183,6 +207,7 @@
         }
         f32x4 part[4];
         {
+            const f32x4 bias6 = *(const f32x4*)(s_b6 + g * 8 + m6 * 4);
             const f32x4 seed = cc == 0 ? bias6 : f32x4{0.f, 0.f, 0.f, 0.f};
 #pragma unroll
             for (int r = 0; r < 4; ++r) part[r] = seed;
@@ -199,13 +224,27 @@
         }
         __syncthreads();
         {
-            float* s_part = (float*)s_l1;
+            float* s_part = (float*)(s_l1 + PART_PIX * 128);
 #pragma unroll
             for (int r = 0; r < 4; ++r) *(f32x4*)(s_part + (((m6 * 4 + cc) * 4 + r) * 64 + lane) * 4) = part[r];
         }
-        __syncthreads();
-        {
-            const float* s_part = (const float*)s_l1;
+        const bool carry_down = more && nxt.carry;
+        u32x4 cp[2];
+        unsigned cp2 = 0u;
+        const unsigned cpo = opaque_u32((unsigned)tid) * 16u;
+        if (carry_down) {
+#pragma unroll
+            for (int k = 0; k < 2; ++k) cp[k] = *(const u32x4*)((const char*)s_l1 + cpo + (CARRY_FROM + k * 512) * 16);
+            if (cpo < 256 * 16u) cp2 = *(const unsigned*)((const char*)s_l1 + (cpo >> 2) + (CARRY_FROM + 1024) * 16);
+        }
+        __syncthreads();
+        if (carry_down) {
+#pragma unroll
+            for (int k = 0; k < 2; ++k) *(u32x4*)((char*)s_l1 + cpo + k * 512 * 16) = cp[k];
+            if (cpo < 256 * 16u) *(unsigned*)((char*)s_l1 + (cpo >> 2) + 1024 * 16) = cp2;
+        }
+        {
+            const float* s_part = (const float*)(s_l1 + PART_PIX * 128);
             const int mr = wave >> 2, rr = wave & 3;
             f32x4 v = *(const f32x4*)(s_part + (((mr * 4 + 0) * 4 + rr) * 64 + lane) * 4);
 #pragma unroll
@@ -216,6 +255,7 @@
             if (oy < OH && ox < OW)
                 *(u32x2*)(a.b1o + ((size_t)(b * OH + oy) * OW + ox) * 32 + g * 8 + mr * 4) = u32x2{relu_pk(pack2(v[0], v[1])), relu_pk(pack2(v[2], v[3]))};
         }
+        cur = nxt;
     }
 }
 
diff --git a/upliftingtabletennis_amd/csrc/conv_stem.h b/upliftingtabletennis_amd/csrc/conv_stem.h
--- a/upliftingtabletennis_amd/csrc/conv_stem.h
+++ b/upliftingtabletennis_amd/csrc/conv_stem.h
@@ -1,5 +1,6 @@
 #pragma once
 #include "conv64.h"
+#include "strip_walk.h"
 
 namespace ttup {
 
@@ -9,7 +10,8 @@
     const bf16_t* w2 = nullptr; const float* b2 = nullptr;
     const bf16_t* w3 = nullptr; const float* b3 = nullptr;
     bf16_t* t2 = nullptr; bf16_t* a1 = nullptr;
-    int H = 0, W = 0, tiles_x = 0, tiles_per_img = 0, total_tiles = 0;
+    int H = 0, W = 0;
+    StripWalk walk;
 };
 
 template <int NF, bool K4 = false>
@@ -21,6 +23,8 @@
     constexpr int W1_U = KS1 * 4 * 64, W2_U = 2 * 9 * 4 * 64;
     constexpr int X_UNITS = NF ? XH * XW * NF : XH * XW * 2;
     constexpr int X_PT = (X_UNITS + 511) / 512;
+    constexpr int X_UNITS_C = X_UNITS / XH * (XH - 2), X_SKIP = X_UNITS / XH * 2;
+    constexpr int CARRY_U = 2 * TW1 * 4, CARRY_FROM = (TH1 - 2) * TW1 * 4;
     extern __shared__ __attribute__((aligned(16))) char smem[];
     bf16_t* s_w1 = (bf16_t*)smem;
     bf16_t* s_w2 = s_w1 + W1_U * 8;
@@ -55,7 +59,9 @@
 #pragma unroll
     for (int dx = 0; dx < 3; ++dx) bB[dx] = s_t1 + lds_off<32, TW1>(0, n + dx, g);
 
-    const int my_tiles = (a.total_tiles - (int)blockIdx.x + (int)gridDim.x - 1) / (int)gridDim.x;
+    const int run_slot = strip_slot((int)blockIdx.x, (int)gridDim.x, a.walk.xcd_deal);
+    const int run_begin = strip_run_begin(run_slot, (int)gridDim.x, a.walk.total);
+    const int my_tiles = strip_run_begin(run_slot + 1, (int)gridDim.x, a.walk.total) - run_begin;
     u32x4 px[NF ? 1 : 2];
     u32x2 pf[NF ? X_PT : 1];
     if (NF) {
@@ -72,13 +78,17 @@
         }
     }
     auto issue = [&](int it) {
-        const TileAt t = tile_at<8, 32, 2>(xcd_tile(blockIdx.x + it * gridDim.x, a.total_tiles), a.tiles_per_img, a.tiles_x);
-        const int b = t.b, gy0 = t.y0, gx0 = t.x0;
+        const StripTile t = strip_tile_at(a.walk, run_begin, it);
+        const int r0 = t.carry ? 2 : 0, xu = t.carry ? X_UNITS_C : X_UNITS;
+        const int b = t.b, gy0 = t.ty * 8 - 2 + r0, gx0 = t.tx * 32 - 2;
         if (NF) {
-            if (gy0 >= 0 && gy0 + XH <= a.H && gx0 >= 0 && gx0 + XW <= a.W) {
+            if (gy0 >= 0 && gy0 + XH - r0 <= a.H && gx0 >= 0 && gx0 + XW <= a.W) {
                 const char* base = (const char*)(a.x0 + (((size_t)b * a.H + gy0) * a.W + gx0) * 4);
 #pragma unroll
-                for (int k = 0; k < X_PT; ++k) pf[k] = *(const u32x2*)(base + opaque_u32(xoff[k]));
+                for (int k = 0; k < X_PT; ++k) {
+                    if ((k + 1) * 512 > X_UNITS_C && tid + k * 512 >= xu) continue;
+                    pf[k] = *(const u32x2*)(base + opaque_u32(xoff[k]));
+                }
                 return;
             }
 #pragma unroll
@@ -87,7 +97,7 @@
                 const int f = u % (NF ? NF : 1), pix = u / (NF ? NF : 1);
                 const int gy = gy0 + pix / XW, gx = gx0 + pix % XW;
                 pf[k] = u32x2{0u, 0u};
-                if (u < X_UNITS && gy >= 0 && gy < a.H && gx >= 0 && gx < a.W)
+                if (u < xu && gy >= 0 && gy < a.H && gx >= 0 && gx < a.W)
                     pf[k] = *(const u32x2*)(a.x0 + (((size_t)(b + f) * a.H + gy) * a.W + gx) * 4);
             }
             return;
@@ -98,20 +108,21 @@
             const int c8 = u & 1, pix = u >> 1;
             const int gy = gy0 + pix / XW, gx = gx0 + pix % XW;
             px[k & (NF ? 0 : 1)] = u32x4{0u, 0u, 0u, 0u};
-            if (u < X_UNITS && gy >= 0 && gy < a.H && gx >= 0 && gx < a.W)
+            if (u < xu && gy >= 0 && gy < a.H && gx >= 0 && gx < a.W)
                 px[k & (NF ? 0 : 1)] = *(const u32x4*)(a.x0 + ((size_t)(b * a.H + gy) * a.W + gx) * 16 + c8 * 8);
         }
     };
-    auto commit = [&]() {
+    auto commit = [&](bool carry) {
+        const int xu = carry ? X_UNITS_C : X_UNITS, skip = carry ? X_SKIP : 0;
         if (NF) {
 #pragma unroll
             for (int k = 0; k < X_PT; ++k) {
                 const int u = tid + k * 512;
-                if (u < X_UNITS) *(u32x2*)(s_x + (u / (NF ? NF : 1)) * XS + (u % (NF ? NF : 1)) * 4) = pf[k];
+                if (u < xu) *(u32x2*)(s_x + ((u + skip) / (NF ? NF : 1)) * XS + (u % (NF ? NF : 1)) * 4) = pf[k];
             }
         } else {
 #pragma unroll
-            for (int k = 0; k < 2; ++k) { const int u = tid + k * 512; if (u < X_UNITS) ((u32x4*)s_x)[u] = px[k & (NF ? 0 : 1)]; }
+            for (int k = 0; k < 2; ++k) { const int u = tid + k * 512; if (u < xu) ((u32x4*)s_x)[u + skip] = px[k & (NF ? 0 : 1)]; }
         }
     };
     auto epilogue = [&](const f32x4 (&acc)[4][2], int b, int oy0, int ox0) __attribute__((always_inline)) {
@@ -143,50 +154,87 @@
     issue(0);
     stage_store_512<W1_U>(s_w1, w1regs, tid);
     stage_store_512<W2_U>(s_w2, w2regs, tid);
-    commit();
+    commit(false);
     if (my_tiles > 1) issue(1);
+    StripTile cur = strip_tile_at(a.walk, run_begin, 0);
     for (int it = 0; it < my_tiles; ++it) {
-        const TileAt tile = tile_at<8, 32>(xcd_tile(blockIdx.x + it * gridDim.x, a.total_tiles), a.tiles_per_img, a.tiles_x);
-        const int b = tile.b, oy0 = tile.y0, ox0 = tile.x0;
+        const int b = cur.b, oy0 = cur.ty * 8, ox0 = cur.tx * 32;
         const bool t1_inside = oy0 >= 1 && oy0 + 9 <= a.H && ox0 >= 1 && ox0 + 33 <= a.W;
         __syncthreads();
-#pragma unroll
-        for (int t = 0; t < 3; ++t) {
-            const int j = wave + 8 * t;
-            if (j >= 22) continue;
-            const int p = j * 16 + n, pc = p < NP1 ? p : NP1 - 1;
-            const int y = pc / TW1, x = pc % TW1;
-            const bf16_t* xb = s_x + (y * XW + x) * XS;
-            f32x4 acc[4] = {b1[0], b1[1], b1[2], b1[3]};
-#pragma unroll
-            for (int s5 = 0; s5 < KS1; ++s5) {
-                bf16x8 bfr;
-                if (K4) {
-                    const u32x2 lo = *(const u32x2*)(xb + koff1[s5]), hi = *(const u32x2*)(xb + koff1[s5] + 4);
-                    bfr = __builtin_bit_cast(bf16x8, u32x4{lo.x, lo.y, hi.x, hi.y});
-                } else bfr = *(const bf16x8*)(xb + koff1[s5]);
+        if (cur.carry && !late) {
+#pragma unroll
+            for (int k = 0; k < 3; ++k) {
+                const int u = tid + k * 256;
+                if (u < 2 * CARRY_U) ((u32x4*)s_t1)[(u / CARRY_U) * (NP1 * 4) + u % CARRY_U] = __builtin_bit_cast(u32x4, acc[k][0]);
+            }
+        }
+        auto x_frag = [&](const bf16_t* xb, int s5) __attribute__((always_inline)) {
+            if (K4) {
+                const u32x2 lo = *(const u32x2*)(xb + koff1[s5]), hi = *(const u32x2*)(xb + koff1[s5] + 4);
+                return __builtin_bit_cast(bf16x8, u32x4{lo.x, lo.y, hi.x, hi.y});
+            }
+            return *(const bf16x8*)(xb + koff1[s5]);
+        };
+        {
+            const int r0 = cur.carry ? 2 : 0;
+#pragma unroll
+            for (int t = 0; t < 3; ++t) {
+                const int j = wave + 8 * t;
+                if (t == 2 && (cur.carry || j >= 22)) continue;
+                const int p = j * 16 + n, pc = p < NP1 ? p : NP1 - 1;
+                const int y = pc / TW1, x = pc % TW1;
+                const bf16_t* xb = s_x + (y * XW + x) * XS + r0 * (XW * XS);
+                f32x4 acc[4] = {b1[0], b1[1], b1[2], b1[3]};
+#pragma unroll
+                for (int s5 = 0; s5 < KS1; ++s5) {
+                    const bf16x8 bfr = x_frag(xb, s5);
+#pragma unroll
+                    for (int m = 0; m < 4; ++m) {
+                        const bf16x8 af = *(const bf16x8*)(s_w1 + ((s5 * 4 + m) * 64 + lane) * 8);
+                        acc[m] = __builtin_amdgcn_mfma_f32_16x16x32_bf16(af, bfr, acc[m], 0, 0, 0);
+                    }
+                }
+                if (p < NP1) {
+                    const int gy = oy0 - 1 + r0 + y, gx = ox0 - 1 + x;
+#pragma unroll
+                    for (int q = 0; q < 2; ++q) {
+                        u32x4 pk = pack8(acc[2 * q], acc[2 * q + 1], true);
+                        if (!t1_inside) {
+                            const bool inside = gy >= 0 && gy < a.H && gx >= 0 && gx < a.W;
+#pragma unroll
+                            for (int i = 0; i < 4; ++i) pk[i] = inside ? pk[i] : 0u;
+                        }
+                        *(u32x4*)(s_t1 + (g >> 1) * (NP1 * 32) + lds_off<32, TW1>(y, x, (g & 1) * 2 + q) + r0 * (TW1 * 32)) = pk;
+                    }
+                }
+            }
+            if (cur.carry) {
+                const unsigned ln = opaque_u32((unsigned)lane);
+                const int n16 = (int)(ln & 15u), g16 = (int)(ln >> 4);
+                constexpr int Y16 = (2 * TW1 + 256) / TW1, X16 = (2 * TW1 + 256) % TW1;
+                static_assert(X16 + 15 < TW1, "group 16 lies in one row");
+                const int x = X16 + n16;
+                const bf16_t* xb = s_x + (Y16 * XW + x) * XS;
+                const int gy = oy0 - 1 + Y16, gx = ox0 - 1 + x;
+                const bool inside = gy >= 0 && gy < a.H && gx >= 0 && gx < a.W;
 #pragma unroll
                 for (int m = 0; m < 4; ++m) {
-                    const bf16x8 af = *(const bf16x8*)(s_w1 + ((s5 * 4 + m) * 64 + lane) * 8);
-                    acc[m] = __builtin_amdgcn_mfma_f32_16x16x32_bf16(af, bfr, acc[m], 0, 0, 0);
-                }
-            }
-            if (p < NP1) {
-                const int gy = oy0 - 1 + y, gx = ox0 - 1 + x;
-#pragma unroll
-                for (int q = 0; q < 2; ++q) {
-                    u32x4 pk = pack8(acc[2 * q], acc[2 * q + 1], true);
-                    if (!t1_inside) {
-                        const bool inside = gy >= 0 && gy < a.H && gx >= 0 && gx < a.W;
-#pragma unroll
-                        for (int i = 0; i < 4; ++i) pk[i] = inside ? pk[i] : 0u;
+                    if (wave != m) continue;
+                    f32x4 acc = b1[m];
+#pragma unroll
+                    for (int s5 = 0; s5 < KS1; ++s5) {
+                        const bf16x8 af = *(const bf16x8*)(s_w1 + ((s5 * 4 + m) * 64 + lane) * 8);
+                        acc = __builtin_amdgcn_mfma_f32_16x16x32_bf16(af, x_frag(xb, s5), acc, 0, 0, 0);
                     }
-                    *(u32x4*)(s_t1 + (g >> 1) * (NP1 * 32) + lds_off<32, TW1>(y, x, (g & 1) * 2 + q)) = pk;
+                    u32x2 pk = u32x2{relu_pk(pack2(acc[0], acc[1])), relu_pk(pack2(acc[2], acc[3]))};
+                    if (!inside) pk = u32x2{0u, 0u};
+                    *(u32x2*)(s_t1 + (g16 >> 1) * (NP1 * 32) + lds_off<32, TW1>(Y16, x, (g16 & 1) * 2 + (m >> 1)) + (m & 1) * 4) = pk;
                 }
             }
         }
         __syncthreads();
-        commit();
+        const StripTile nxt = it + 1 < my_tiles ? strip_tile_at(a.walk, run_begin, it + 1) : StripTile{cur.b, cur.ty, cur.tx, 0};
+        commit(nxt.carry != 0);
         if (it + 2 < my_tiles) issue(it + 2);
         if (STAGGER && late && pending) epilogue(acc, eb, eoy0, eox0);
 #pragma unroll
@@ -195,6 +243,14 @@
         conv64_tile_mfma(acc, bB, s_w2, wave, lane);
         if (STAGGER && late) { eb = b; eoy0 = oy0; eox0 = ox0; pending = true; }
         else epilogue(acc, b, oy0, ox0);
+        if (nxt.carry && !late) {
+#pragma unroll
+            for (int k = 0; k < 3; ++k) {
+                const int u = tid + k * 256;
+                if (u < 2 * CARRY_U) acc[k][0] = __builtin_bit_cast(f32x4, ((const u32x4*)s_t1)[(u / CARRY_U) * (NP1 * 4) + CARRY_FROM + u % CARRY_U]);
+            }
+        }
+        cur = nxt;
     }
     if (STAGGER && late && pending) epilogue(acc, eb, eoy0, eox0);
 }
diff --git a/upliftingtabletennis_amd/csrc/strip_walk.h b/upliftingtabletennis_amd/csrc/strip_walk.h
--- /dev/null
+++ b/upliftingtabletennis_amd/csrc/strip_walk.h
@@ -0,0 +1,40 @@
+#pragma once
+
+#if defined(__HIPCC__) || defined(__CUDACC__)
+#define TTUP_HD __host__ __device__ inline
+#else
+#define TTUP_HD inline
+#endif
+
+namespace ttup {
+
+struct StripWalk {
+    int total = 0, tiles_x = 0, tiles_y = 0;
+    int xcd_deal = 1;
+    int carry = 1;
+};
+struct StripTile { int b, ty, tx, carry; };
+
+TTUP_HD int strip_slot(int wg, int grid, int xcd_deal) {
+    const int main = grid & ~7;
+    return xcd_deal && wg < main ? (wg & 7) * (main >> 3) + (wg >> 3) : wg;
+}
+TTUP_HD int strip_run_begin(int s, int grid, int total) {
+    const int q = total / grid, r = total % grid;
+    return s * q + (s < r ? s : r);
+}
+TTUP_HD int strip_run_len(const StripWalk& w, int wg, int grid) {
+    const int s = strip_slot(wg, grid, w.xcd_deal);
+    return strip_run_begin(s + 1, grid, w.total) - strip_run_begin(s, grid, w.total);
+}
+TTUP_HD StripTile strip_tile_at(const StripWalk& w, int begin, int it) {
+    const int seq = begin + it, per_img = w.tiles_x * w.tiles_y;
+    const int b = seq / per_img, t = seq % per_img;
+    const int ty = t % w.tiles_y;
+    return StripTile{b, ty, t / w.tiles_y, (w.carry && it > 0 && ty > 0) ? 1 : 0};
+}
+TTUP_HD StripTile strip_tile(const StripWalk& w, int wg, int grid, int it) {
+    return strip_tile_at(w, strip_run_begin(strip_slot(wg, grid, w.xcd_deal), grid, w.total), it);
+}
+
+}
diff --git a/upliftingtabletennis_amd/csrc/wasb_net.h b/upliftingtabletennis_amd/csrc/wasb_net.h
--- a/upliftingtabletennis_amd/csrc/wasb_net.h
+++ b/upliftingtabletennis_amd/csrc/wasb_net.h
@@ -51,6 +51,7 @@
     int t_input = -1, t_out = -1;
     int t_frames = -1;
     bool frames_mode = false;
+    ttup::StripOpts strip;
     float* head_w_dev = nullptr; float* head_b_dev = nullptr; float head_bias = 0.f;
     int n_out = 1;
     float* heat_scratch = nullptr;
diff --git a/upliftingtabletennis_amd/csrc/wasb_net.hip b/upliftingtabletennis_amd/csrc/wasb_net.hip
--- a/upliftingtabletennis_amd/csrc/wasb_net.hip
+++ b/upliftingtabletennis_amd/csrc/wasb_net.hip
@@ -52,7 +52,7 @@
         const Tensor& s = net->tensors[op.src0];
         const bool fm = net->frames_mode && net->t_frames >= 0 && op.conv1f >= 0;
         const int rc = launch_stem(net->convs[fm ? op.conv1f : op.conv], net->convs[op.conv2], net->convs[op.conv3], fm ? net->tensors[net->t_frames].ptr : s.ptr,
-                                   net->tensors[op.dst].ptr, net->tensors[op.dst2].ptr, mb, s.h, s.w, st, fm ? net->in_ch / 3 : 0);
+                                   net->tensors[op.dst].ptr, net->tensors[op.dst2].ptr, mb, s.h, s.w, st, fm ? net->in_ch / 3 : 0, net->strip);
         if (rc) return rc;
     } else if (op.kind == Op::UPSUM_HEAD) {
         return TTUP_OK;
@@ -73,7 +73,7 @@
     } else if (op.kind == Op::BNECK_TRANS) {
         const Tensor& s = net->tensors[op.src0];
         const int rc = launch_bneck_trans(net->convs[op.conv], net->convs[op.conv2], net->convs[op.conv3], s.ptr, net->tensors[op.src1].ptr,
-                                          net->tensors[op.dst].ptr, net->tensors[op.dst2].ptr, mb, s.h, s.w, st);
+                                          net->tensors[op.dst].ptr, net->tensors[op.dst2].ptr, mb, s.h, s.w, st, net->strip);
         if (rc) return rc;
     } else {
         const Tensor& d = net->tensors[op.dst];
@@ -285,6 +285,8 @@
     GraphSwitches sw;
     sw.fuse = !env_set("TTUP_NO_FUSE"); sw.fuse_sum = !env_set("TTUP_NO_FUSE_SUM"); sw.fuse_lin = !env_set("TTUP_NO_FUSE_LIN");
     sw.pair = !env_set("TTUP_NO_PAIR"); sw.stem = !env_set("TTUP_NO_STEM"); sw.frames_mode = !env_set("TTUP_NO_FRAMES_MODE");
+    net->strip.carry = !env_set("TTUP_NO_CARRY"); net->strip.xcd_deal = env_ll("TTUP_STRIP_DEAL", 1) != 0;
+    net->strip.max_wgs = (int)env_ll("TTUP_PERSIST_WGS", 0);
     const GraphPlan plan = build_graph(folded, in_ch, net->n_out, height, width, net->micro, dtype, sw);
     if (plan.rc) return plan.rc;
     net->ops = plan.ops; net->taps = plan.taps;
```

Result: slower. 2151 (-1.9%).
